# pkorus/neural-imaging

Hardware: AMD Instinct MI355X
Metric: patches/s (fwd+bwd) ISP->JPEG->FAN @256^2 (higher is better)
Workload: dtype bf16; 1 GPU; c4 = train_manipulation UNet->[native,sharpen:1,resample:50,gaussian:0.83,jpeg:80]->dJPEG(QF80,soft)->FAN, ds none, trainable nip+fan, lambda_nip 0.1; raw_patch=128, batch_per_gpu=64, global_batch=64, parallelism=dp1, world_size=1, hip_graph=False

## Files before the change

### include/nimg.h

```cpp
#ifndef NIMG_H
#define NIMG_H

#include <stddef.h>
#include <stdint.h>

#ifdef __cplusplus
extern "C" {
#endif

#define NIMG_OK 0
#define NIMG_ERR_ARG (-1)
#define NIMG_ERR_LAUNCH (-2)
#define NIMG_ERR_WORKSPACE (-3)

#define NIMG_BF16_IN 1
#define NIMG_BF16_OUT 2
#define NIMG_BF16_MASK 4
#define NIMG_BF16_DZ 8
#define NIMG_D2S_OUT 16
#define NIMG_MASK_CONV 128
#define NIMG_COPY_LRELU 64
#define NIMG_S2D_OUT 32
#define NIMG_UNPOOL_OUT 512
#define NIMG_D2S_CONVT 1024
#define NIMG_POOL_ALSO 256

#define NIMG_ABI_VERSION 8
int nimg_abi_version(void);

#define NIMG_ROUND_ROUND 0
#define NIMG_ROUND_SOFT 1
#define NIMG_ROUND_SIN 2
#define NIMG_ROUND_HARMONIC 3
#define NIMG_ROUND_IDENTITY 4

int nimg_djpeg_fwd(const float* x, float* y, const float* qtab, uint8_t* mask, int16_t* idx, float* xdq,
                   int n, int h, int w, int rounding, void* stream);
int nimg_djpeg_bwd(const float* x, const float* gy, const uint8_t* mask, const float* qtab, float* gx,
                   int n, int h, int w, int rounding, void* stream);
size_t nimg_djpeg_dq_workspace_bytes(int n, int h, int w);
int nimg_djpeg_bwd_dq(const float* x, const float* gy, const uint8_t* mask, const float* qtab, float* gx, float* dq,
                      int n, int h, int w, int rounding, int accumulate, void* workspace, size_t workspace_bytes,
                      void* stream);
size_t nimg_djpeg_sub_workspace_bytes(int n, int h, int w, int hs, int vs, int with_dq);
int nimg_djpeg_sub_fwd(const float* x, float* y, const float* qtab, uint8_t* mask, int16_t* idx, float* xdq,
                       int n, int h, int w, int hs, int vs, int rounding, void* workspace, size_t workspace_bytes,
                       void* stream);
int nimg_djpeg_sub_bwd(const float* x, const float* gy, const uint8_t* mask, const float* qtab, float* gx,
                       float* dq , int n, int h, int w, int hs, int vs, int rounding, int accumulate,
                       void* workspace, size_t workspace_bytes, void* stream);
int nimg_jpeg_qtable(int quality, int channel, float* out64);

int nimg_conv2d_fwd(const float* in1, int c1, const float* in2, int c2, const float* w, const float* bias,
                    float* out1, int o1, float* out2, int o2, const float* act_mask, int n, int h, int wd, int ks,
                    int stride, int pad_t, int pad_l, int pad_mode, int hout, int wout, int act, float alpha,
                    void* stream);
int nimg_conv_flip_weights(const float* w, float* wt, int ks_h, int ks_w, int cin, int cout, void* stream);
size_t nimg_conv2d_wgrad_workspace_bytes(int cin, int cout, int ks_h, int ks_w, int n, int hout, int wout);
int nimg_conv2d_wgrad(const float* in1, int c1, const float* in2, int c2, const float* dz, int cout, float* dw,
                      float* db, int n, int h, int wd, int ks, int stride, int pad_t, int pad_l, int pad_mode, int hout,
                      int wout, int accumulate, void* workspace, size_t workspace_bytes, void* stream);
size_t nimg_bias_grad_workspace_bytes(long npix, int cout);
int nimg_bias_grad(const float* dz, float* db, long npix, int cout, int accumulate, void* workspace,
                   size_t workspace_bytes, void* stream);
int nimg_bias_grad_ex(const float* dz, float* db, long npix, int cout, int accumulate, void* workspace,
                      size_t workspace_bytes, int flags, void* stream);
int nimg_convt2x2_fwd(const float* x, const float* w, const float* bias, float* y, int n, int h, int wd, int cin,
                      int cout, void* stream);

int nimg_maxpool2_fwd(const float* x, float* y, int n, int h, int w, int c, void* stream);
int nimg_maxpool2_bwd(const float* dp, const float* yact, const float* add, float* dz, int n, int h, int w, int c,
                      int apply_lrelu_mask, float alpha, void* stream);
int nimg_maxpool2_fwd_bf16(const void* x, void* y, int n, int h, int w, int c, void* stream);
int nimg_maxpool2_bwd_bf16(const void* dp, const void* yact, const void* add, void* dz, int n, int h, int w, int c,
                           int apply_lrelu_mask, float alpha, void* stream);
int nimg_conv2d_pool_fwd(const float* in, int cin, const float* w, const float* bias, float* pool_out,
                         unsigned char* pool_idx, int cout, int n, int h, int wd, int ks, int act, float alpha,
                         void* stream);
int nimg_conv2d_pool_fwd_bf16(const float* in, int cin, const float* w, const void* wb, const float* bias,
                              float* pool_out, unsigned char* pool_idx, int cout, int n, int h, int wd, int ks, int act,
                              float alpha, void* stream);
int nimg_maxpool2_unpool(const float* dp, const unsigned char* idx, const float* pooled, float* dz, int n, int ho, int wo,
                         int c, int apply_lrelu_mask, float alpha, void* stream);
int nimg_d2s_clip_fwd(const float* x, float* y, int n, int h, int w, int cout, float scale, float shift, int clip,
                      void* stream);
int nimg_d2s_clip_bwd(const float* dy, float* dx, int n, int h, int w, int cout, float scale, void* stream);
int nimg_lrelu_bwd(const float* dy, const float* yact, float* dz, long count, float alpha, void* stream);
int nimg_add(const float* a, const float* b, float* out, long count, void* stream);
int nimg_add_n(const float* const* inputs, int n_inputs, float* out, long count, void* stream);
int nimg_avgpool_fwd(const float* x, float* y, int n, int h, int w, int c, int factor, void* stream);
int nimg_avgpool_bwd(const float* dy, float* dx, int n, int h, int w, int c, int factor, void* stream);

size_t nimg_mse255_workspace_bytes(void);
int nimg_mse255(const float* a, const float* b, float* loss, float* grad_a, long count, float grad_scale,
                int accumulate, void* workspace, size_t workspace_bytes, void* stream);
size_t nimg_mae255_workspace_bytes(void);
int nimg_mae255(const float* a, const float* b, float* loss, float* grad_a, long count, float grad_scale,
                int accumulate, void* workspace, size_t workspace_bytes, void* stream);
size_t nimg_ssim_loss_workspace_bytes(int n, int h, int w, int c, int with_grad);
int nimg_ssim_loss(const float* y, const float* t, float* loss, float* grad_y, int n, int h, int w, int c,
                   float max_val, const float* gauss_win, float grad_scale, int accumulate, void* workspace,
                   size_t workspace_bytes, void* stream);
int nimg_mse255_sum_s2d3(const float* const* parts, int n_parts, const float* y, const float* target, float* loss, float* dz,
                         int n, int h, int w, float grad_scale, void* workspace, size_t workspace_bytes, void* stream);
size_t nimg_ssim_workspace_bytes(int n);
int nimg_ssim(const float* a, const float* b, float* out, int n, int h, int w, int c, int mode, float max_val,
              const float* gauss_win, void* workspace, size_t workspace_bytes, void* stream);
int nimg_fan_head_fwd(const float* act, const float* w, const float* b, const int* labels, float* gap, float* probs,
                      float* loss_per, float* dlogits, int n, int hw, int c, int k, float loss_scale, void* stream);
int nimg_fan_head_bwd(const float* act, const float* gap, const float* w, const float* dlogits,
                      const float* loss_per, float* dact, float* dw, float* db, float* loss, int n, int hw, int c,
                      int k, float loss_scale, float alpha, void* stream);
int nimg_adam_step(float* params, const float* grads, float* m, float* v, long count, float lr, float beta1,
                   float beta2, float eps, int step, float grad_scale, const int* skip_flag, void* stream);
int nimg_adam_step_dev(float* params, const float* grads, float* m, float* v, long count, const float* lr_t, float beta1,
                       float beta2, float eps, float grad_scale, const int* skip_flag, void* stream);
int nimg_nan_flag(const float* g, long count, int* flag, void* stream);
int nimg_int_words(int* dst, const int* src, long n, int value, int mode, void* stream);
int nimg_float_fill(float* dst, long n, float value, void* stream);

#define NIMG_TICKET_BYTES (64 * 1024)
#define NIMG_TICKET_STREAMS 16
int nimg_bind_tickets(void* stream, void* buf, size_t bytes);

int nimg_stream_create_cu_mask(int n_cus, void** stream);
int nimg_stream_destroy(void* stream);

int nimg_head_fused_ok(int hw, int c);
int nimg_head_fwd(const void* x, const void* wimg, const float* bias, unsigned* mask, unsigned* mask_p, float* gap, int n, int hw,
                  int c, float alpha, void* stream);
size_t nimg_head_wgrad_workspace_bytes(int n, int c);
int nimg_head_wgrad(const void* x, const unsigned* mask_p, const float* dlogits, const float* wdense, int k, float* dw, float* db,
                    int n, int hw, int c, float alpha, int accumulate, void* workspace, size_t workspace_bytes, void* stream);
int nimg_head_dgrad(const unsigned* mask, const float* dlogits, const float* wdense, int k, const void* wimg_t,
                    const void* in_mask, void* dx, int n, int hw, int c, float alpha, void* stream);
int nimg_head_dact(const unsigned* mask, const float* dlogits, const float* wdense, int k, void* dact, int n, int hw, int c,
                   float alpha, void* stream);
int nimg_fan_dense_fwd(const float* gap, const float* w, const float* b, const int* labels, float* probs, float* loss_per,
                       float* dlogits, int n, int c, int k, float loss_scale, void* stream);
int nimg_fan_dense_bwd(const float* gap, const float* dlogits, const float* loss_per, float* dw, float* db, float* loss, int n,
                       int c, int k, float loss_scale, void* stream);

int nimg_constrained_kernel_fwd(const float* kernel, float* nf, int ks, int channels, float strength, void* stream);
int nimg_constrained_kernel_bwd(const float* kernel, const float* dnf, float* dkernel, int ks, int channels,
                                float strength, void* stream);
int nimg_fold_pad(const float* dpad, float* dx, int n, int h, int w, int c, int pad, int pad_mode, void* stream);

int nimg_gaussian_fwd(const float* x, float* y, uint8_t* mask, const float* gk25, int n, int h, int w, int clip,
                      void* stream);
int nimg_gaussian_bwd(const float* dy, const uint8_t* mask, float* dx, const float* gk25, int n, int h, int w,
                      void* stream);
int nimg_dwfilter_fwd(const float* x, float* y, uint8_t* mask, const float* taps, int k, int pad_mode, int n, int h, int w,
                      int clip, void* stream);
int nimg_dwfilter_bwd(const float* dy, const uint8_t* mask, float* dx, const float* taps, int k, int pad_mode, int n, int h,
                      int w, void* stream);
int nimg_sharpen_fwd(const float* x, float* y, float* aux_hsv, uint8_t* mask, const float* gk9, int n, int h, int w,
                     void* stream);
int nimg_sharpen_bwd(const float* x, const float* dy, float* aux_hsv, const uint8_t* mask, float* dx,
                     const float* gk9, int n, int h, int w, void* stream);
int nimg_sparse_axis_apply(const float* in, float* out, const int* rowptr, const int* col, const float* val, int n,
                           int hin, int win, int c, int axis, int out_size, void* stream);

size_t nimg_ssim_planes_workspace_bytes(int n, int c);
int nimg_ssim_planes(const float* y, const float* t, int n, int h, int w, int c, float max_val, const float* gauss_win,
                     float* mean_ssim, float* mean_cs, float* maps, int which_maps, void* workspace,
                     size_t workspace_bytes, void* stream);
int nimg_msssim_combine(const float* values, const float* items, int scales, int planes, float* loss, float* coef,
                        void* stream);
int nimg_ssim_maps_grad(const float* y, const float* t, const float* maps, const float* coef, float* grad_y, int n,
                        int h, int w, int c, const float* gauss_win, float grad_scale, int accumulate, void* stream);
size_t nimg_msssim_workspace_bytes(int n, int h, int w, int c);
int nimg_msssim(const float* a, const float* b, int n, int h, int w, int c, float max_val, const float* gauss_win, double* out,
                void* workspace, size_t workspace_bytes, void* stream);

int nimg_patch_stats(const uint8_t* rgb, int n_images, int h, int w, const int* image_idx, const int* cand_xy, int b,
                     int attempts, int patch, double* var_out, double* mean_out, void* stream);
int nimg_patch_select(const int* cand_xy, const float* uniforms, const double* var, const double* mean, int b,
                      int attempts, int max_attempts, int mode, int* chosen_xy, int* attempts_used, void* stream);
int nimg_patch_gather(const uint16_t* raw, const uint8_t* rgb, int n_images, int h, int w, const int* image_idx,
                      const int* xy, int b, int patch, float* x_out, float* y_out, void* stream);

int nimg_affine(const float* x, float* y, long count, float a, float b, void* stream);
int nimg_lrelu_fwd(const float* x, float* y, long count, float alpha, void* stream);
int nimg_tanh_fwd(const float* x, float* y, long count, void* stream);
int nimg_tanh_bwd(const float* dy, const float* y, float* dx, long count, void* stream);
int nimg_clip01(const float* x, float* y, long count, void* stream);
int nimg_pad2d(const float* x, float* y, int n, int h, int w, int c, int pad, int pad_mode, void* stream);
int nimg_isp_residual_fwd(const float* x, const float* f, const float* alpha, float* y, long count, int clip,
                          void* stream);
long nimg_isp_residual_workspace_bytes(void);
int nimg_isp_residual_bwd(const float* dy, const float* f, const float* alpha, float* df, float* dalpha,
                          float* workspace, long count, int accumulate, void* stream);
int nimg_mask_scale(const float* x, const uint8_t* keep, float* y, long count, float scale, void* stream);
size_t nimg_conv5_dgrad_sparse_image_bytes(int cin, int cout);
int nimg_conv5_dgrad_sparse_weights(const float* w, void* image, int cin, int cout, void* stream);
int nimg_conv5_dgrad_sparse(const void* g, const unsigned char* idx, int cout, const void* image, void* out, int cin,
                            const void* act_mask, int n, int h, int wd, float alpha, int flags, void* stream);
int nimg_conv2d_fwd_bf16_res(const float* in1, int c1, const void* wb, const float* bias, float* out1, int o1,
                             const float* act_mask, const float* residual, void* out_bf16_copy, int n, int h, int wd, int ks,
                             int stride, int pad_t, int pad_l, int pad_mode, int hout, int wout, int act, float alpha, int flags,
                             void* stream);
int nimg_conv2d_fwd_bf16_unpool(const void* in_pooled, const unsigned char* in_idx, int c1, const void* wb, const float* bias,
                                float* out1, int o1, const float* act_mask, int n, int h, int w_, int ks, int pad_t, int pad_l,
                                int hout, int wout, int act, float alpha, int flags, void* stream);
int nimg_conv2d_wgrad_bf16_unpool(const void* in, int cin, const void* g, const unsigned char* idx, int cout, float* dw, float* db,
                                  int n, int h, int w_, int ks, int accumulate, void* workspace, size_t workspace_bytes,
                                  void* stream);
int nimg_conv2d_wgrad_bf16_deferred(const void* in1, int c1, const void* in2, int c2, const void* dz, const unsigned char* idx,
                                    int cout, float* dw, float* db, int n, int h, int wd, int ks, int stride, int pad_t, int pad_l,
                                    int pad_mode, int hout, int wout, void* workspace, size_t workspace_bytes, int flags,
                                    void* entry, void* stream);
int nimg_conv2d_wgrad_bf16_chained(const void* in1, int c1, const void* in2, int c2, const void* dz, const unsigned char* idx,
                                   int cout, float* dw, float* db, int n, int h, int wd, int ks, int stride, int pad_t, int pad_l,
                                   int pad_mode, int hout, int wout, void* workspace, size_t workspace_bytes, int flags,
                                   const void* pre_entry, void* entry, void* stream);
size_t nimg_reduce_entry_bytes(void);
int nimg_reduce_batch_max(void);
int nimg_reduce_slabs_batch(const void* entries, int n, void* stream);

int nimg_conv5c3_bf16(const float* in, const float* w, float* out, int n, int h, int wd, void* stream);
int nimg_cconv3(const float* in, const float* w, float* out_f32, void* out_c4, int n, int h, int w_, int pad_mode,
                void* stream);
int nimg_cconv3_dgrad_border(const float* dc, const float* nf, float* dx, int n, int h, int w_, void* stream);
int nimg_conv1_pool_fwd_c4(const void* c4, const float* w, const float* bias, void* pooled, unsigned char* pool_idx, int n,
                           int h, int w_, float alpha, int out_bf16, void* stream);
size_t nimg_conv1_wgrad_c4_workspace_bytes(void);
int nimg_conv1_wgrad_c4(const void* c4, const void* g, const unsigned char* pool_idx, float* dw, float* db, int n, int h, int w_,
                        int g_bf16, int accumulate, void* workspace, size_t workspace_bytes, void* stream);
int nimg_conv1_dgrad_pooled(const void* g, const unsigned char* pool_idx, const float* w, float* dc, int n, int h, int w_,
                            int g_bf16, void* stream);
int nimg_confusion_accumulate(const float* probs, const int* labels, int* pred, unsigned long long* conf, int n, int k,
                              void* stream);
int nimg_sigmoid_fwd(const float* x, float* y, long count, void* stream);
int nimg_sigmoid_bwd(const float* dy, const float* y, float* dx, long count, void* stream);
int nimg_activation_fwd(const float* x, float* y, long count, int kind, float alpha, void* stream);
int nimg_activation_bwd(const float* dy, const float* y, float* dx, long count, int kind, float alpha, void* stream);
int nimg_gamma_ste_fwd(const float* x, float* y, long count, float lo, float hi, float exponent, void* stream);
int nimg_gamma_ste_bwd(const float* x, const float* dy, float* dx, long count, float lo, float hi, float exponent,
                       void* stream);
int nimg_s2d2_affine_bf16(const float* x, void* y, int n, int h, int w, int c, int cp, float a, float b, void* stream);
int nimg_s2d_conv_weights(const float* w5, float* w3, int cin, int cp, int cout, void* stream);
int nimg_s2d_conv_weights_bwd(const float* dw3, float* dw5, int cin, int cp, int cout, int accumulate, void* stream);
int nimg_d2s2_scale(const float* xs, float* x, int n, int h, int w, int c, int cp, float scale, void* stream);
int nimg_zero_insert2(const float* in, float* out, int n, int h, int w, int c, void* stream);
size_t nimg_latent_workspace_bytes(int codebook_size);
int nimg_latent_fwd(const float* z, const float* scale, const float* codebook, int codebook_size, float v,
                    float gamma, int soft_codebook, float* latent, float* entropy, long count, long count_global,
                    void* workspace, size_t workspace_bytes, int finalize, void* stream);
int nimg_latent_entropy_finalize(int codebook_size, long count_global, float* entropy, void* workspace, void* stream);
int nimg_latent_bwd(const float* z, const float* scale, const float* latent, const float* dlatent,
                    float entropy_coef, const float* codebook, int codebook_size, float v, float gamma,
                    int soft_codebook, float* dz, float* dscale, int accumulate_dscale, long count, void* workspace,
                    size_t workspace_bytes, void* stream);
size_t nimg_l2_loss_workspace_bytes(void);
int nimg_l2_loss(const float* target, const float* y, float* loss, float* grad_y, long count, float grad_scale,
                 int accumulate, void* workspace, size_t workspace_bytes, void* stream);

size_t nimg_conv_weights_bf16_bytes(int ks_h, int ks_w, int cin, int cout, int mode);
int nimg_conv_weights_bf16(const float* w, void* wb, int ks_h, int ks_w, int cin, int cout, int mode, void* stream);
int nimg_conv2d_wgrad_pooled_bf16(const float* in, int cin, const float* g, const unsigned char* idx, int cout,
                                  float* dw, float* db, int n, int h, int wd, int ks, int accumulate, void* workspace,
                                  size_t workspace_bytes, void* stream);
int nimg_conv2d_dgrad_fewin_pooled_bf16(const float* g, const unsigned char* idx, const float* w, float* out, int ci,
                                        int cz, int n, int h, int wd, int ks, void* stream);
int nimg_conv2d_fwd_bf16_ex(const float* in1, int c1, const float* in2, int c2, const void* wb, const float* bias,
                            float* out1, int o1, float* out2, int o2, const float* act_mask, int n, int h, int wd,
                            int ks, int stride, int pad_t, int pad_l, int pad_mode, int hout, int wout, int act,
                            float alpha, int flags, void* stream);
int nimg_conv2d_wgrad_bf16_ex(const float* in1, int c1, const float* in2, int c2, const float* dz, int cout, float* dw,
                              float* db, int n, int h, int wd, int ks, int stride, int pad_t, int pad_l, int pad_mode,
                              int hout, int wout, int accumulate, void* workspace, size_t workspace_bytes, int flags,
                              void* stream);
int nimg_conv2d_pool_fwd_bf16_ex(const float* in, int cin, const float* w, const void* wb, const float* bias,
                                 float* pool_out, unsigned char* pool_idx, int cout, int n, int h, int wd, int ks,
                                 int act, float alpha, int flags, void* stream);
int nimg_conv2d_fwd_pool_also_bf16(const float* in, int cin, const void* wb, const float* bias, float* out, float* pool_out,
                                   unsigned char* pool_idx, int cout, int n, int h, int wd, int act, float alpha, void* stream);
#define NIMG_ROWS_F32_OUT 1
int nimg_conv3_rows_bf16(const void* in1, int c1, const void* in2, int c2, const void* wb, const float* bias, const void* mask,
                         void* out, void* out2, void* pool_out, int n, int h, int wd, int cout, int act, float alpha, int flags,
                         void* stream);
int nimg_conv3_rows_d2s_bf16(const void* in, int c1, const void* wb, const float* bias, float* y, int n, int h, int wd, void* stream);
int nimg_conv3_rows_c4_bf16(const float* in, const float* w, const float* bias, void* out, int n, int h, int wd, int act, float alpha,
                            void* stream);

int nimg_conv2d_dgrad_unpool_out_bf16(const float* dz, int c1, const void* wb, const float* act, const float* skip, float* out,
                                      int cout, int n, int h, int wd, int apply_mask, float alpha, void* stream);
int nimg_conv2d_wgrad_pooled_bf16_ex(const float* in, int cin, const float* g, const unsigned char* idx, int cout,
                                     float* dw, float* db, int n, int h, int wd, int ks, int accumulate, void* workspace,
                                     size_t workspace_bytes, int flags, void* stream);
int nimg_conv2d_dgrad_fewin_pooled_bf16_ex(const float* g, const unsigned char* idx, const float* w, float* out, int ci,
                                           int cz, int n, int h, int wd, int ks, int flags, void* stream);
int nimg_maxpool2_unpool_ex(const float* dp, const unsigned char* idx, const float* pooled, float* dz, int n, int ho,
                            int wo, int c, int apply_lrelu_mask, float alpha, int flags, void* stream);
int nimg_convt2x2_fwd_bf16(const float* x, const void* wb, const float* bias, float* y, int n, int h, int wd, int cin,
                           int cout, void* stream);
int nimg_convt2x2_fwd_bf16_ex(const float* x, const void* wb, const float* bias, float* y, int n, int h, int wd, int cin,
                              int cout, int flags, void* stream);
int nimg_conv_weights_bf16_batch(const void* table, int n_entries, void* stream);
int nimg_conv2d_fwd_bf16(const float* in1, int c1, const float* in2, int c2, const void* wb, const float* bias,
                         float* out1, int o1, float* out2, int o2, const float* act_mask, int n, int h, int wd,
                         int ks, int stride, int pad_t, int pad_l, int pad_mode, int hout, int wout, int act,
                         float alpha, void* stream);
size_t nimg_conv2d_wgrad_bf16_workspace_bytes(int cin, int cout, int ks_h, int ks_w, int n, int hout, int wout);
int nimg_conv2d_wgrad_bf16(const float* in1, int c1, const float* in2, int c2, const float* dz, int cout, float* dw,
                           float* db, int n, int h, int wd, int ks, int stride, int pad_t, int pad_l, int pad_mode,
                           int hout, int wout, int accumulate, void* workspace, size_t workspace_bytes, void* stream);

int nimg_conv2d_fwd_smallc_bf16(const float* in, int cin, const float* w, const float* bias, float* out, int cout,
                                int n, int h, int wd, int ks, int pad_mode, int act, float alpha, void* stream);
int nimg_conv2d_fwd_smallc_bf16_ex(const float* in, int cin, const float* w, const float* bias, float* out, int cout,
                                   int n, int h, int wd, int ks, int pad_mode, int act, float alpha, int flags, void* stream);
int nimg_conv2d_dgrad_fewin_bf16(const float* dz, const float* w, float* out, int ci, int cz, int n, int h, int wd,
                                 int ks, void* stream);

int nimg_awgn_fwd(const float* x, const float* noise, float* y, uint8_t* mask, long count, float strength,
                  void* stream);
int nimg_awgn_bwd(const float* x, const float* noise, const float* dy, const uint8_t* mask, float* dx, long count,
                  float strength, void* stream);
int nimg_gamma_fwd(const float* x, float* y, long count, float gamma, void* stream);
int nimg_gamma_bwd(const float* x, const float* dy, float* dx, long count, float gamma, void* stream);
int nimg_median_fwd(const float* x, float* y, uint8_t* sel, int n, int h, int w, int kernel, void* stream);
int nimg_median_bwd(const float* dy, const uint8_t* sel, float* dx, int n, int h, int w, int kernel, void* stream);

#define NIMG_L3IC_E_READ 1
#define NIMG_L3IC_E_LANES 2
#define NIMG_L3IC_E_RANGE 4
#define NIMG_L3IC_E_SYMBOL 8
#define NIMG_L3IC_E_FREQ 16
#define NIMG_L3IC_E_VARINT 32
#define NIMG_L3IC_E_ODD 64
#define NIMG_L3IC_E_UNUSED 128
#define NIMG_L3IC_E_STATE 256
#define NIMG_L3IC_E_RLE 512
size_t nimg_l3ic_workspace_bytes(int n_streams, int n_sym);
int nimg_l3ic_quantise(const float* z, const float* codebook, int codebook_size, uint8_t* idx, int* err, int n, int h,
                       int w, int c, void* stream);
int nimg_l3ic_encode(const uint8_t* idx, int n_streams, int n_sym, uint8_t* out, uint32_t* lengths, uint32_t* hist,
                     uint32_t* freq, void* workspace, size_t workspace_bytes, void* stream);
int nimg_l3ic_decode(const uint8_t* data, const uint32_t* offsets, const uint32_t* lengths, const float* codebook,
                     int codebook_size, float* z, uint32_t* err, int n, int h, int w, int c, void* stream);

size_t nimg_jpeg_workspace_bytes(int n, int h, int w, int hs, int vs);
int nimg_jpeg_transform(const void* x, int is_u8, int n, int h, int w, int hs, int vs, int quality, int16_t* coef, void* workspace,
                        size_t workspace_bytes, void* stream);
int nimg_jpeg_encode(const int16_t* coef, int n, int h, int w, int hs, int vs, uint8_t* out, size_t out_capacity, uint32_t* lengths,
// ... 57 lines not shown
```

### neural-imaging_amd/_lib.py

```python
import ctypes
import os
from ctypes import c_float, c_int, c_long, c_size_t, c_void_p

_HERE = os.path.dirname(os.path.abspath(__file__))
LIB_PATH = os.environ.get('NIMG_LIBPATH') or os.path.join(_HERE, 'libnimg.so')

P = c_void_p

PROTOTYPES = {
    'nimg_abi_version': (c_int, []),
    'nimg_djpeg_fwd': (c_int, [P, P, P, P, P, P, c_int, c_int, c_int, c_int, P]),
    'nimg_djpeg_bwd': (c_int, [P, P, P, P, P, c_int, c_int, c_int, c_int, P]),
    'nimg_djpeg_dq_workspace_bytes': (c_size_t, [c_int, c_int, c_int]),
    'nimg_djpeg_bwd_dq': (c_int, [P, P, P, P, P, P, c_int, c_int, c_int, c_int, c_int, P, c_size_t, P]),
    'nimg_djpeg_sub_workspace_bytes': (c_size_t, [c_int, c_int, c_int, c_int, c_int, c_int]),
    'nimg_djpeg_sub_fwd': (c_int, [P, P, P, P, P, P, c_int, c_int, c_int, c_int, c_int, c_int, P, c_size_t, P]),
    'nimg_djpeg_sub_bwd': (c_int, [P, P, P, P, P, P, c_int, c_int, c_int, c_int, c_int, c_int, c_int, P, c_size_t, P]),
    'nimg_jpeg_qtable': (c_int, [c_int, c_int, P]),
    'nimg_conv2d_fwd': (c_int, [P, c_int, P, c_int, P, P, P, c_int, P, c_int, P, c_int, c_int, c_int, c_int, c_int,
                                c_int, c_int, c_int, c_int, c_int, c_int, c_float, P]),
    'nimg_conv_flip_weights': (c_int, [P, P, c_int, c_int, c_int, c_int, P]),
    'nimg_conv2d_wgrad_workspace_bytes': (c_size_t, [c_int, c_int, c_int, c_int, c_int, c_int, c_int]),
    'nimg_conv2d_wgrad': (c_int, [P, c_int, P, c_int, P, c_int, P, P, c_int, c_int, c_int, c_int, c_int, c_int, c_int,
                                  c_int, c_int, c_int, c_int, P, c_size_t, P]),
    'nimg_bias_grad_workspace_bytes': (c_size_t, [c_long, c_int]),
    'nimg_bias_grad': (c_int, [P, P, c_long, c_int, c_int, P, c_size_t, P]),
    'nimg_bias_grad_ex': (c_int, [P, P, c_long, c_int, c_int, P, c_size_t, c_int, P]),
    'nimg_convt2x2_fwd': (c_int, [P, P, P, P, c_int, c_int, c_int, c_int, c_int, P]),
    'nimg_maxpool2_fwd': (c_int, [P, P, c_int, c_int, c_int, c_int, P]),
    'nimg_maxpool2_bwd': (c_int, [P, P, P, P, c_int, c_int, c_int, c_int, c_int, c_float, P]),
    'nimg_maxpool2_fwd_bf16': (c_int, [P, P, c_int, c_int, c_int, c_int, P]),
    'nimg_maxpool2_bwd_bf16': (c_int, [P, P, P, P, c_int, c_int, c_int, c_int, c_int, c_float, P]),
    'nimg_conv2d_pool_fwd': (c_int, [P, c_int, P, P, P, P, c_int, c_int, c_int, c_int, c_int, c_int, c_float, P]),
    'nimg_conv2d_pool_fwd_bf16': (c_int, [P, c_int, P, P, P, P, P, c_int, c_int, c_int, c_int, c_int, c_int, c_float,
                                          P]),
    'nimg_maxpool2_unpool': (c_int, [P, P, P, P, c_int, c_int, c_int, c_int, c_int, c_float, P]),
    'nimg_d2s_clip_fwd': (c_int, [P, P, c_int, c_int, c_int, c_int, c_float, c_float, c_int, P]),
    'nimg_d2s_clip_bwd': (c_int, [P, P, c_int, c_int, c_int, c_int, c_float, P]),
    'nimg_lrelu_bwd': (c_int, [P, P, P, c_long, c_float, P]),
    'nimg_add': (c_int, [P, P, P, c_long, P]),
    'nimg_add_n': (c_int, [P, c_int, P, c_long, P]),
    'nimg_avgpool_fwd': (c_int, [P, P, c_int, c_int, c_int, c_int, c_int, P]),
    'nimg_avgpool_bwd': (c_int, [P, P, c_int, c_int, c_int, c_int, c_int, P]),
    'nimg_mse255_workspace_bytes': (c_size_t, []),
    'nimg_mse255': (c_int, [P, P, P, P, c_long, c_float, c_int, P, c_size_t, P]),
    'nimg_mse255_sum_s2d3': (c_int, [P, c_int, P, P, P, P, c_int, c_int, c_int, c_float, P, c_size_t, P]),
    'nimg_fan_head_fwd': (c_int, [P, P, P, P, P, P, P, P, c_int, c_int, c_int, c_int, c_float, P]),
    'nimg_fan_head_bwd': (c_int, [P, P, P, P, P, P, P, P, P, c_int, c_int, c_int, c_int, c_float, c_float, P]),
    'nimg_adam_step': (c_int, [P, P, P, P, c_long, c_float, c_float, c_float, c_float, c_int, c_float, P, P]),
    'nimg_adam_step_dev': (c_int, [P, P, P, P, c_long, P, c_float, c_float, c_float, c_float, P, P]),
    'nimg_conv3_rows_bf16': (c_int, [P, c_int, P, c_int, P, P, P, P, P, P, c_int, c_int, c_int, c_int, c_int, c_float, c_int, P]),
    'nimg_conv3_rows_d2s_bf16': (c_int, [P, c_int, P, P, P, c_int, c_int, c_int, P]),
    'nimg_conv2d_wgrad_bf16_deferred': (c_int, [P, c_int, P, c_int, P, P, c_int, P, P, c_int, c_int, c_int, c_int, c_int, c_int, c_int,
                                                c_int, c_int, c_int, P, c_size_t, c_int, P, P]),
    'nimg_conv2d_wgrad_bf16_chained': (c_int, [P, c_int, P, c_int, P, P, c_int, P, P, c_int, c_int, c_int, c_int, c_int, c_int, c_int,
                                               c_int, c_int, c_int, P, c_size_t, c_int, P, P, P]),
    'nimg_reduce_entry_bytes': (c_size_t, []),
    'nimg_reduce_batch_max': (c_int, []),
    'nimg_reduce_slabs_batch': (c_int, [P, c_int, P]),
    'nimg_conv3_rows_c4_bf16': (c_int, [P, P, P, P, c_int, c_int, c_int, c_int, c_float, P]),
    'nimg_nan_flag': (c_int, [P, c_long, P, P]),
    'nimg_int_words': (c_int, [P, P, c_long, c_int, c_int, P]),
    'nimg_float_fill': (c_int, [P, c_long, c_float, P]),
    'nimg_bind_tickets': (c_int, [P, P, c_size_t]),
    'nimg_stream_create_cu_mask': (c_int, [c_int, P]),
    'nimg_stream_destroy': (c_int, [P]),
    'nimg_head_fused_ok': (c_int, [c_int, c_int]),
    'nimg_head_fwd': (c_int, [P, P, P, P, P, P, c_int, c_int, c_int, c_float, P]),
    'nimg_head_wgrad_workspace_bytes': (c_size_t, [c_int, c_int]),
    'nimg_head_wgrad': (c_int, [P, P, P, P, c_int, P, P, c_int, c_int, c_int, c_float, c_int, P, c_size_t, P]),
    'nimg_head_dgrad': (c_int, [P, P, P, c_int, P, P, P, c_int, c_int, c_int, c_float, P]),
    'nimg_head_dact': (c_int, [P, P, P, c_int, P, c_int, c_int, c_int, c_float, P]),
    'nimg_fan_dense_fwd': (c_int, [P, P, P, P, P, P, P, c_int, c_int, c_int, c_float, P]),
    'nimg_fan_dense_bwd': (c_int, [P, P, P, P, P, P, c_int, c_int, c_int, c_float, P]),
    'nimg_constrained_kernel_fwd': (c_int, [P, P, c_int, c_int, c_float, P]),
    'nimg_constrained_kernel_bwd': (c_int, [P, P, P, c_int, c_int, c_float, P]),
    'nimg_fold_pad': (c_int, [P, P, c_int, c_int, c_int, c_int, c_int, c_int, P]),
    'nimg_gaussian_fwd': (c_int, [P, P, P, P, c_int, c_int, c_int, c_int, P]),
    'nimg_gaussian_bwd': (c_int, [P, P, P, P, c_int, c_int, c_int, P]),
    'nimg_dwfilter_fwd': (c_int, [P, P, P, P, c_int, c_int, c_int, c_int, c_int, c_int, P]),
    'nimg_dwfilter_bwd': (c_int, [P, P, P, P, c_int, c_int, c_int, c_int, c_int, P]),
    'nimg_sharpen_fwd': (c_int, [P, P, P, P, P, c_int, c_int, c_int, P]),
    'nimg_sharpen_bwd': (c_int, [P, P, P, P, P, P, c_int, c_int, c_int, P]),
    'nimg_affine': (c_int, [P, P, c_long, c_float, c_float, P]),
    'nimg_lrelu_fwd': (c_int, [P, P, c_long, c_float, P]),
    'nimg_zero_insert2': (c_int, [P, P, c_int, c_int, c_int, c_int, P]),
    'nimg_s2d2_affine_bf16': (c_int, [P, P, c_int, c_int, c_int, c_int, c_int, c_float, c_float, P]),
    'nimg_s2d_conv_weights': (c_int, [P, P, c_int, c_int, c_int, P]),
    'nimg_s2d_conv_weights_bwd': (c_int, [P, P, c_int, c_int, c_int, c_int, P]),
    'nimg_d2s2_scale': (c_int, [P, P, c_int, c_int, c_int, c_int, c_int, c_float, P]),
    'nimg_latent_workspace_bytes': (c_size_t, [c_int]),
    'nimg_latent_fwd': (c_int, [P, P, P, c_int, c_float, c_float, c_int, P, P, c_long, c_long, P, c_size_t, c_int, P]),
    'nimg_latent_entropy_finalize': (c_int, [c_int, c_long, P, P, P]),
    'nimg_latent_bwd': (c_int, [P, P, P, P, c_float, P, c_int, c_float, c_float, c_int, P, P, c_int, c_long, P,
                                c_size_t, P]),
    'nimg_l2_loss_workspace_bytes': (c_size_t, []),
    'nimg_l2_loss': (c_int, [P, P, P, P, c_long, c_float, c_int, P, c_size_t, P]),
    'nimg_conv_weights_bf16_bytes': (c_size_t, [c_int, c_int, c_int, c_int, c_int]),
    'nimg_conv_weights_bf16': (c_int, [P, P, c_int, c_int, c_int, c_int, c_int, P]),
    'nimg_conv2d_fwd_bf16': (c_int, [P, c_int, P, c_int, P, P, P, c_int, P, c_int, P, c_int, c_int, c_int, c_int,
                                     c_int, c_int, c_int, c_int, c_int, c_int, c_int, c_float, P]),
    'nimg_conv2d_wgrad_bf16_workspace_bytes': (c_size_t, [c_int, c_int, c_int, c_int, c_int, c_int, c_int]),
    'nimg_conv2d_wgrad_bf16': (c_int, [P, c_int, P, c_int, P, c_int, P, P, c_int, c_int, c_int, c_int, c_int, c_int,
                                       c_int, c_int, c_int, c_int, c_int, P, c_size_t, P]),
    'nimg_conv2d_wgrad_pooled_bf16': (c_int, [P, c_int, P, P, c_int, P, P, c_int, c_int, c_int, c_int, c_int, P, c_size_t,
                                              P]),
    'nimg_conv2d_dgrad_fewin_pooled_bf16': (c_int, [P, P, P, P, c_int, c_int, c_int, c_int, c_int, c_int, P]),
    'nimg_ssim_workspace_bytes': (c_size_t, [c_int]),
    'nimg_ssim': (c_int, [P, P, P, c_int, c_int, c_int, c_int, c_int, c_float, P, P, c_size_t, P]),
    'nimg_tanh_fwd': (c_int, [P, P, c_long, P]),
    'nimg_tanh_bwd': (c_int, [P, P, P, c_long, P]),
    'nimg_clip01': (c_int, [P, P, c_long, P]),
    'nimg_isp_residual_fwd': (c_int, [P, P, P, P, c_long, c_int, P]),
    'nimg_isp_residual_workspace_bytes': (c_long, []),
    'nimg_isp_residual_bwd': (c_int, [P, P, P, P, P, P, c_long, c_int, P]),
    'nimg_activation_fwd': (c_int, [P, P, c_long, c_int, c_float, P]),
    'nimg_activation_bwd': (c_int, [P, P, P, c_long, c_int, c_float, P]),
    'nimg_sigmoid_fwd': (c_int, [P, P, c_long, P]),
    'nimg_sigmoid_bwd': (c_int, [P, P, P, c_long, P]),
    'nimg_gamma_ste_fwd': (c_int, [P, P, c_long, c_float, c_float, c_float, P]),
    'nimg_gamma_ste_bwd': (c_int, [P, P, P, c_long, c_float, c_float, c_float, P]),
    'nimg_mae255_workspace_bytes': (c_size_t, []),
    'nimg_mae255': (c_int, [P, P, P, P, c_long, c_float, c_int, P, c_size_t, P]),
    'nimg_ssim_loss_workspace_bytes': (c_size_t, [c_int, c_int, c_int, c_int, c_int]),
    'nimg_ssim_loss': (c_int, [P, P, P, P, c_int, c_int, c_int, c_int, c_float, P, c_float, c_int, P, c_size_t, P]),
    'nimg_patch_stats': (c_int, [P, c_int, c_int, c_int, P, P, c_int, c_int, c_int, P, P, P]),
    'nimg_patch_select': (c_int, [P, P, P, P, c_int, c_int, c_int, c_int, P, P, P]),
    'nimg_patch_gather': (c_int, [P, P, c_int, c_int, c_int, P, P, c_int, c_int, P, P, P]),
    'nimg_mask_scale': (c_int, [P, P, P, c_long, c_float, P]),
    'nimg_conv5_dgrad_sparse_image_bytes': (c_size_t, [c_int, c_int]),
    'nimg_conv5_dgrad_sparse_weights': (c_int, [P, P, c_int, c_int, P]),
    'nimg_conv5_dgrad_sparse': (c_int, [P, P, c_int, P, P, c_int, P, c_int, c_int, c_int, c_float, c_int, P]),
    'nimg_conv2d_fwd_bf16_res': (c_int, [P, c_int, P, P, P, c_int, P, P, P, c_int, c_int, c_int, c_int, c_int, c_int, c_int, c_int, c_int,
                                 c_int, c_int, c_float, c_int, P]),
    'nimg_conv2d_fwd_bf16_unpool': (c_int, [P, P, c_int, P, P, P, c_int, P, c_int, c_int, c_int, c_int, c_int, c_int, c_int,
                                            c_int, c_int, c_float, c_int, P]),
    'nimg_conv2d_wgrad_bf16_unpool': (c_int, [P, c_int, P, P, c_int, P, P, c_int, c_int, c_int, c_int, c_int, P, c_size_t, P]),
    'nimg_cconv3': (c_int, [P, P, P, P, c_int, c_int, c_int, c_int, P]),
    'nimg_conv5c3_bf16': (c_int, [P, P, P, c_int, c_int, c_int, P]),
    'nimg_cconv3_dgrad_border': (c_int, [P, P, P, c_int, c_int, c_int, P]),
    'nimg_conv1_pool_fwd_c4': (c_int, [P, P, P, P, P, c_int, c_int, c_int, c_float, c_int, P]),
    'nimg_conv1_wgrad_c4_workspace_bytes': (c_size_t, []),
    'nimg_conv1_wgrad_c4': (c_int, [P, P, P, P, P, c_int, c_int, c_int, c_int, c_int, P, c_size_t, P]),
    'nimg_conv1_dgrad_pooled': (c_int, [P, P, P, P, c_int, c_int, c_int, c_int, P]),
    'nimg_confusion_accumulate': (c_int, [P, P, P, P, c_int, c_int, P]),
    'nimg_ssim_planes_workspace_bytes': (c_size_t, [c_int, c_int]),
    'nimg_ssim_planes': (c_int, [P, P, c_int, c_int, c_int, c_int, c_float, P, P, P, P, c_int, P, c_size_t, P]),
    'nimg_msssim_combine': (c_int, [P, P, c_int, c_int, P, P, P]),
    'nimg_ssim_maps_grad': (c_int, [P, P, P, P, P, c_int, c_int, c_int, c_int, P, c_float, c_int, P]),
    'nimg_pad2d': (c_int, [P, P, c_int, c_int, c_int, c_int, c_int, c_int, P]),
    'nimg_conv2d_fwd_bf16_ex': (c_int, [P, c_int, P, c_int, P, P, P, c_int, P, c_int, P, c_int, c_int, c_int, c_int, c_int,
                                        c_int, c_int, c_int, c_int, c_int, c_int, c_float, c_int, P]),
    'nimg_conv2d_wgrad_bf16_ex': (c_int, [P, c_int, P, c_int, P, c_int, P, P, c_int, c_int, c_int, c_int, c_int, c_int,
                                          c_int, c_int, c_int, c_int, c_int, P, c_size_t, c_int, P]),
    'nimg_conv2d_pool_fwd_bf16_ex': (c_int, [P, c_int, P, P, P, P, P, c_int, c_int, c_int, c_int, c_int, c_int, c_float,
                                             c_int, P]),
    'nimg_conv2d_dgrad_unpool_out_bf16': (c_int, [P, c_int, P, P, P, P, c_int, c_int, c_int, c_int, c_int, c_float, P]),
    'nimg_conv2d_fwd_pool_also_bf16': (c_int, [P, c_int, P, P, P, P, P, c_int, c_int, c_int, c_int, c_int, c_float, P]),
    'nimg_conv2d_wgrad_pooled_bf16_ex': (c_int, [P, c_int, P, P, c_int, P, P, c_int, c_int, c_int, c_int, c_int, P,
                                                 c_size_t, c_int, P]),
    'nimg_conv2d_dgrad_fewin_pooled_bf16_ex': (c_int, [P, P, P, P, c_int, c_int, c_int, c_int, c_int, c_int, c_int, P]),
    'nimg_maxpool2_unpool_ex': (c_int, [P, P, P, P, c_int, c_int, c_int, c_int, c_int, c_float, c_int, P]),
    'nimg_conv_weights_bf16_batch': (c_int, [P, c_int, P]),
    'nimg_convt2x2_fwd_bf16': (c_int, [P, P, P, P, c_int, c_int, c_int, c_int, c_int, P]),
    'nimg_convt2x2_fwd_bf16_ex': (c_int, [P, P, P, P, c_int, c_int, c_int, c_int, c_int, c_int, P]),
    'nimg_conv2d_fwd_smallc_bf16': (c_int, [P, c_int, P, P, P, c_int, c_int, c_int, c_int, c_int, c_int, c_int,
                                            c_float, P]),
    'nimg_conv2d_fwd_smallc_bf16_ex': (c_int, [P, c_int, P, P, P, c_int, c_int, c_int, c_int, c_int, c_int, c_int,
                                               c_float, c_int, P]),
    'nimg_conv2d_dgrad_fewin_bf16': (c_int, [P, P, P, c_int, c_int, c_int, c_int, c_int, c_int, P]),
    'nimg_awgn_fwd': (c_int, [P, P, P, P, c_long, c_float, P]),
    'nimg_awgn_bwd': (c_int, [P, P, P, P, P, c_long, c_float, P]),
    'nimg_gamma_fwd': (c_int, [P, P, c_long, c_float, P]),
    'nimg_gamma_bwd': (c_int, [P, P, P, c_long, c_float, P]),
    'nimg_median_fwd': (c_int, [P, P, P, c_int, c_int, c_int, c_int, P]),
    'nimg_median_bwd': (c_int, [P, P, P, c_int, c_int, c_int, c_int, P]),
    'nimg_sparse_axis_apply': (c_int, [P, P, P, P, P, c_int, c_int, c_int, c_int, c_int, c_int, P]),
    'nimg_l3ic_workspace_bytes': (c_size_t, [c_int, c_int]),
    'nimg_l3ic_quantise': (c_int, [P, P, c_int, P, P, c_int, c_int, c_int, c_int, P]),
    'nimg_l3ic_encode': (c_int, [P, c_int, c_int, P, P, P, P, P, c_size_t, P]),
    'nimg_l3ic_decode': (c_int, [P, P, P, P, c_int, P, P, c_int, c_int, c_int, c_int, P]),
    'nimg_jpeg_workspace_bytes': (c_size_t, [c_int, c_int, c_int, c_int, c_int]),
    'nimg_jpeg_transform': (c_int, [P, c_int, c_int, c_int, c_int, c_int, c_int, c_int, P, P, c_size_t, P]),
    'nimg_jpeg_encode': (c_int, [P, c_int, c_int, c_int, c_int, c_int, P, c_size_t, P, P, c_size_t, P]),
    'nimg_jpeg_reconstruct': (c_int, [P, c_int, c_int, c_int, c_int, c_int, c_int, P, P, c_size_t, P]),
    'nimg_jpeg_transform_items': (c_int, [P, c_int, c_int, c_int, c_int, c_int, c_int, P, c_int, P, P, P, c_size_t, P]),
    'nimg_jpeg_reconstruct_items': (c_int, [P, c_int, c_int, c_int, c_int, c_int, P, P, P, P, c_size_t, P]),
    'nimg_jpeg_decode_workspace_bytes': (c_size_t, [c_int, c_int, c_int, c_int, c_int, c_size_t, c_int]),
    'nimg_jpeg_decode': (c_int, [P, P, P, c_int, c_int, c_int, c_int, c_int, c_int, P, P, P, P, c_size_t, P]),
    'nimg_jpeg_reconstruct_tables': (c_int, [P, c_int, c_int, c_int, c_int, c_int, P, P, c_int, P, c_size_t, P]),
    'nimg_jpeg_histogram': (c_int, [P, c_int, c_int, c_int, c_int, c_int, P, P]),
    'nimg_jpeg_optimal_tables': (c_int, [P, c_int, P, P, P]),
    'nimg_jpeg_encode_tables_workspace_bytes': (c_size_t, [c_int, c_int, c_int, c_int, c_int]),
    'nimg_jpeg_encode_tables': (c_int, [P, c_int, c_int, c_int, c_int, c_int, P, P, c_size_t, P, P, P, c_size_t, P]),
    'nimg_jpeg_transform_tables': (c_int, [P, c_int, c_int, c_int, c_int, c_int, c_int, P, c_int, P, P, P, c_size_t, P]),
    'nimg_jpeg_tables_from_float': (c_int, [P, c_int, c_int, P, P, P]),
    'nimg_jpeg_encode_restart_workspace_bytes': (c_size_t, [c_int, c_int, c_int, c_int, c_int, c_int]),
    'nimg_jpeg_encode_restart': (c_int, [P, c_int, c_int, c_int, c_int, c_int, c_int, P, c_size_t, P, P, c_size_t, P]),
    'nimg_jpeg_histogram_restart': (c_int, [P, c_int, c_int, c_int, c_int, c_int, c_int, P, P]),
    'nimg_jpeg_encode_tables_restart_workspace_bytes': (c_size_t, [c_int, c_int, c_int, c_int, c_int, c_int]),
    'nimg_jpeg_encode_tables_restart': (c_int, [P, c_int, c_int, c_int, c_int, c_int, c_int, P, P, c_size_t, P, P, P, c_size_t, P]),
    'nimg_jpeg_decode_restart_workspace_bytes': (c_size_t, [c_int, c_int, c_int, c_int, c_int, c_int, c_size_t, c_int]),
    'nimg_jpeg_decode_restart': (c_int, [P, P, P, c_int, c_int, c_int, c_int, c_int, c_int, c_int, P, P, P, P, c_size_t, P]),
    'nimg_msssim_workspace_bytes': (c_size_t, [c_int, c_int, c_int, c_int]),
    'nimg_msssim': (c_int, [P, P, c_int, c_int, c_int, c_int, c_float, P, P, P, c_size_t, P]),
    'nimg_conv1_pool_fwd_c4_sign': (c_int, [P, P, P, P, P, P, c_int, c_int, c_int, c_float, c_int, P]),
    'nimg_conv2d_pool_sign_ok': (c_int, [c_int, c_int, c_int, c_int, c_int, c_int, c_int]),
    'nimg_conv2d_pool_fwd_bf16_sign': (c_int, [P, c_int, P, P, P, P, P, P, c_int, c_int, c_int, c_int, c_int, c_int, c_float,
                                               c_int, P]),
    'nimg_conv2d_fwd_bf16_unpool_sign': (c_int, [P, P, c_int, P, P, P, c_int, P, P, c_int, c_int, c_int, c_int, c_int, c_int, c_int,
                                                 c_int, c_int, c_float, c_int, P]),
}

ERRORS = {-1: 'NIMG_ERR_ARG (invalid argument / unsupported configuration)',
          -2: 'NIMG_ERR_LAUNCH (HIP kernel launch failed)',
          -3: 'NIMG_ERR_WORKSPACE (workspace too small)'}

_lib = None


ABI_VERSION = 8
TICKET_BYTES = 64 * 1024


def load():
    global _lib
    if _lib is not None:
        return _lib
    if not os.path.isfile(LIB_PATH):
        raise RuntimeError('libnimg.so not found at {} - build it with neural-imaging_amd/csrc/build.sh '
                           '(or __graft_entry__.build()); there is no CPU fallback'.format(LIB_PATH))
    import torch
    lib = ctypes.CDLL(LIB_PATH)
    for name, (res, args) in PROTOTYPES.items():
        fn = getattr(lib, name)
        fn.restype = res
        fn.argtypes = args
    if lib.nimg_abi_version() != ABI_VERSION:
        raise RuntimeError('libnimg.so at {} has ABI version {}, this binding was written against {} - rebuild it '
                           '(neural-imaging_amd/csrc/build.sh)'.format(LIB_PATH, lib.nimg_abi_version(), ABI_VERSION))
    _lib = lib
    return lib


def call(name, *args):
    rc = getattr(load(), name)(*args)
    if rc != 0:
        raise RuntimeError('{} failed: {}'.format(name, ERRORS.get(rc, rc)))
    return rc
```

### neural-imaging_amd/csrc/djpeg.h

```cpp
#pragma once
#include <type_traits>
#include "common.h"

namespace nimg {
namespace dj {

constexpr int STRIP_PX = 64;
constexpr int ROW_STRIDE = 196;
constexpr int STAGE_F = 8 * ROW_STRIDE;

__device__ __forceinline__ void wave_sync() { __builtin_amdgcn_wave_barrier(); }

__device__ constexpr float kF[8][8] = {
    {0.3536f, 0.3536f, 0.3536f, 0.3536f, 0.3536f, 0.3536f, 0.3536f, 0.3536f},
    {0.4904f, 0.4157f, 0.2778f, 0.0975f, -0.0975f, -0.2778f, -0.4157f, -0.4904f},
    {0.4619f, 0.1913f, -0.1913f, -0.4619f, -0.4619f, -0.1913f, 0.1913f, 0.4619f},
    {0.4157f, -0.0975f, -0.4904f, -0.2778f, 0.2778f, 0.4904f, 0.0975f, -0.4157f},
    {0.3536f, -0.3536f, -0.3536f, 0.3536f, 0.3536f, -0.3536f, -0.3536f, 0.3536f},
    {0.2778f, -0.4904f, 0.0975f, 0.4157f, -0.4157f, -0.0975f, 0.4904f, -0.2778f},
    {0.1913f, -0.4619f, 0.4619f, -0.1913f, -0.1913f, 0.4619f, -0.4619f, 0.1913f},
    {0.0975f, -0.2778f, 0.4157f, -0.4904f, 0.4904f, -0.4157f, 0.2778f, -0.0975f}};

__device__ constexpr float kCF[3][4] = {{0.0f, 0.299f, 0.587f, 0.114f},
                                        {128.0f, -0.168736f, -0.331264f, 0.5f},
                                        {128.0f, 0.5f, -0.418688f, -0.081312f}};
__device__ constexpr float kCI[3][4] = {{(float)(-1.402 * 128), 1.0f, 0.0f, 1.402f},
                                        {(float)(1.058272 * 128), 1.0f, -0.344136f, -0.714136f},
                                        {(float)(-1.772 * 128), 1.0f, 1.772f, 0.0f}};

__device__ __forceinline__ void dct_fwd8(const float (&in)[8], float (&out)[8]) {
#pragma unroll
    for (int k = 0; k < 8; ++k) {
        float acc = in[0] * kF[k][0];
#pragma unroll
        for (int m = 1; m < 8; ++m) acc = __builtin_fmaf(in[m], kF[k][m], acc);
        out[k] = acc;
    }
}
__device__ __forceinline__ void dct_inv8(const float (&in)[8], float (&out)[8]) {
#pragma unroll
    for (int m = 0; m < 8; ++m) {
        float acc = in[0] * kF[0][m];
#pragma unroll
        for (int k = 1; k < 8; ++k) acc = __builtin_fmaf(in[k], kF[k][m], acc);
        out[m] = acc;
    }
}

struct Task {
    int n, by, x0;
    bool valid;
};

__device__ __forceinline__ Task decode_task(long task, long n_tasks, int hb, int strips) {
    Task t;
    t.valid = task < n_tasks;
    const long tt = t.valid ? task : 0;
    t.x0 = (int)(tt % strips) * STRIP_PX;
    t.by = (int)((tt / strips) % hb);
    t.n = (int)(tt / ((long)strips * hb));
    return t;
}

typedef float f32x4 __attribute__((ext_vector_type(4)));
__device__ __forceinline__ void fetch_strip(const float* __restrict__ src, f32x4 (&pre)[6], const Task& t, int h, int w,
                                            int lane) {
    const int strip_f = min(STRIP_PX, w - t.x0) * 3;
#pragma unroll
    for (int it = 0; it < 6; ++it) {
        const int idx = it * 64 + lane;
        const int row = idx / 48, c4 = idx % 48;
        if (t.valid && c4 * 4 < strip_f)
            pre[it] = *reinterpret_cast<const f32x4*>(src + (((long)t.n * h + t.by * 8 + row) * w + t.x0) * 3 + c4 * 4);
    }
}
__device__ __forceinline__ void commit_strip(float* lds, const f32x4 (&pre)[6], int lane) {
#pragma unroll
    for (int it = 0; it < 6; ++it) {
        const int idx = it * 64 + lane;
        *reinterpret_cast<f32x4*>(lds + (idx / 48) * ROW_STRIDE + (idx % 48) * 4) = pre[it];
    }
}

__device__ __forceinline__ void store_strip(float* __restrict__ dst, const float* lds, const Task& t, int h, int w,
                                            int lane) {
    const int strip_f = min(STRIP_PX, w - t.x0) * 3;
#pragma unroll
    for (int it = 0; it < 6; ++it) {
        const int idx = it * 64 + lane;
        const int row = idx / 48, c4 = idx % 48;
        if (t.valid && c4 * 4 < strip_f) {
            const float4 v = *reinterpret_cast<const float4*>(lds + row * ROW_STRIDE + c4 * 4);
            *reinterpret_cast<float4*>(dst + (((long)t.n * h + t.by * 8 + row) * w + t.x0) * 3 + c4 * 4) = v;
        }
    }
}

__device__ __forceinline__ void read_row24(const float* lds, int b, int r, float (&px)[24]) {
    const float4* p = reinterpret_cast<const float4*>(lds + r * ROW_STRIDE + b * 24);
#pragma unroll
    for (int k = 0; k < 6; ++k) {
        const float4 v = p[k];
        px[4 * k + 0] = v.x; px[4 * k + 1] = v.y; px[4 * k + 2] = v.z; px[4 * k + 3] = v.w;
    }
}
__device__ __forceinline__ void write_row24(float* lds, int b, int r, const float (&px)[24]) {
    float4* p = reinterpret_cast<float4*>(lds + r * ROW_STRIDE + b * 24);
#pragma unroll
    for (int k = 0; k < 6; ++k) p[k] = make_float4(px[4 * k], px[4 * k + 1], px[4 * k + 2], px[4 * k + 3]);
}

template <int NC>
__device__ __forceinline__ void transpose_tiles(float* tile, int b, int r, float (&v)[NC][8]) {
#pragma unroll
    for (int c = 0; c < NC; ++c)
#pragma unroll
        for (int k = 0; k < 8; ++k) tile[((c * 8 + b) * 8 + r) * 9 + k] = v[c][k];
    wave_sync();
#pragma unroll
    for (int c = 0; c < NC; ++c)
#pragma unroll
        for (int k = 0; k < 8; ++k) v[c][k] = tile[((c * 8 + b) * 8 + k) * 9 + r];
    wave_sync();
}

enum { Q_RINT = 0, Q_SIN = 1, Q_HARMONIC = 2, Q_IDENTITY = 3 };
__host__ __device__ constexpr int fwd_mode(int rounding) {
    return rounding == NIMG_ROUND_SIN ? Q_SIN : rounding == NIMG_ROUND_HARMONIC ? Q_HARMONIC
         : rounding == NIMG_ROUND_IDENTITY ? Q_IDENTITY : Q_RINT;
}
template <int QMODE>
__device__ __forceinline__ float quantise(float u) {
    if constexpr (QMODE == Q_RINT) return rintf(u);
    else if constexpr (QMODE == Q_SIN) return u - sinpif(2.0f * (u - rintf(u))) * 0.15915494309189535f;
    else if constexpr (QMODE == Q_HARMONIC) return u - sinpif(2.0f * (u - rintf(u))) * 0.3183098861837907f;
    else return u;
}
enum { G_ZERO = 0, G_SOFT = 1, G_HARMONIC = 2, G_ONE = 3 };
__host__ __device__ constexpr int bwd_mode(int rounding) {
    return rounding == NIMG_ROUND_ROUND ? G_ZERO : rounding == NIMG_ROUND_HARMONIC ? G_HARMONIC
         : rounding == NIMG_ROUND_IDENTITY ? G_ONE : G_SOFT;
}
template <int GMODE>
__device__ __forceinline__ float quantise_grad(float u) {
    if constexpr (GMODE == G_ZERO) return 0.0f;
    else if constexpr (GMODE == G_ONE) return 1.0f;
    else {
        const float c = __builtin_amdgcn_cosf(__builtin_amdgcn_fractf(u));
        return GMODE == G_SOFT ? 1.0f - c : 1.0f - 2.0f * c;
    }
}

template <bool EXACT>
__device__ __forceinline__ float div_q(float x, float q, float rc) {
    if constexpr (EXACT) return x / q;
    const float y0 = x * rc;
    const float r = __builtin_fmaf(-y0, q, x);
    return __builtin_fmaf(r, rc, y0);
}

__device__ __forceinline__ void colour_fwd(const float (&px)[24], float (&ycc)[3][8]) {
#pragma unroll
    for (int j = 0; j < 8; ++j) {
        const float r = 255.0f * px[3 * j], g = 255.0f * px[3 * j + 1], bb = 255.0f * px[3 * j + 2];
#pragma unroll
        for (int c = 0; c < 3; ++c) {
            float acc = kCF[c][0];
            acc = __builtin_fmaf(r, kCF[c][1], acc);
            acc = __builtin_fmaf(g, kCF[c][2], acc);
            acc = __builtin_fmaf(bb, kCF[c][3], acc);
            ycc[c][j] = acc - 127.0f;
        }
    }
}

__device__ __forceinline__ bool stage_tables(const float* __restrict__ qtab, float* qT, int* flag) {
    const int tid = threadIdx.x;
    if (tid == 0) *flag = 1;
    __syncthreads();
    if (tid < 192) {
        const float q = qtab[tid];
        const int c = tid >> 6, u = (tid >> 3) & 7, r = tid & 7;
        qT[(c * 8 + r) * 8 + u] = q;
        qT[192 + (c * 8 + r) * 8 + u] = 1.0f / q;
        if (!(q >= 1.0f && q <= 255.0f && q == rintf(q))) *flag = 0;
    }
    __syncthreads();
    return __builtin_amdgcn_readfirstlane(*flag) != 0;
}
__device__ __forceinline__ void read_tables(const float* qT, int c, int r, float (&q)[8], float (&rc)[8]) {
#pragma unroll
    for (int k = 0; k < 2; ++k) {
        const float4 a = *reinterpret_cast<const float4*>(qT + (c * 8 + r) * 8 + 4 * k);
        const float4 b = *reinterpret_cast<const float4*>(qT + 192 + (c * 8 + r) * 8 + 4 * k);
        q[4 * k] = a.x; q[4 * k + 1] = a.y; q[4 * k + 2] = a.z; q[4 * k + 3] = a.w;
        rc[4 * k] = b.x; rc[4 * k + 1] = b.y; rc[4 * k + 2] = b.z; rc[4 * k + 3] = b.w;
    }
}

}
}
```

### neural-imaging_amd/csrc/djpeg.hip

```cpp
#include "djpeg.h"

namespace {

using namespace nimg;
using namespace nimg::dj;

constexpr int TILE_F = 3 * 8 * 72;
constexpr int WAVE_LDS_F = (STAGE_F > TILE_F ? STAGE_F : TILE_F);
constexpr int WAVES_PER_BLOCK = 4;
#ifndef DJ_FWD_WGS
#define DJ_FWD_WGS 4
#endif
#ifndef DJ_BWD_WGS
#define DJ_BWD_WGS 3
#endif

__device__ __forceinline__ void transpose24(float* tile, int b, int r, float (&v)[3][8]) { transpose_tiles<3>(tile, b, r, v); }

template <int QMODE, bool EXACT>
__device__ __forceinline__ void quantise_columns(float (&v)[3][8], const float* qT, const Task& t, int b, int r, int hb, int wb,
                                                 int16_t* __restrict__ idx, float* __restrict__ xdq) {
#pragma unroll
    for (int c = 0; c < 3; ++c) {
        float X[8], q[8], rc[8];
        dct_fwd8(v[c], X);
        read_tables(qT, c, r, q, rc);
#pragma unroll
        for (int u = 0; u < 8; ++u) {
            const float qi = quantise<QMODE>(div_q<EXACT>(X[u], q[u], rc[u]));
            X[u] = qi * q[u];
            if (idx || xdq) {
                const long o = ((((long)t.n * 3 + c) * hb + t.by) * wb + (t.x0 / 8 + b)) * 64 + u * 8 + r;
                if (idx) idx[o] = (int16_t)qi;
                if (xdq) xdq[o] = X[u];
            }
        }
        dct_inv8(X, v[c]);
    }
}

template <int QMODE>
__global__ __launch_bounds__(256, DJ_FWD_WGS) void djpeg_fwd_kernel(const float* __restrict__ x, float* __restrict__ y,
                                                        const float* __restrict__ qtab, uint8_t* __restrict__ mask,
                                                        int16_t* __restrict__ idx, float* __restrict__ xdq, int n,
                                                        int h, int w) {
    extern __shared__ __attribute__((aligned(16))) float smem[];
    const int wave = threadIdx.x >> 6, lane = threadIdx.x & 63;
    const int b = lane >> 3, r = lane & 7;
    float* lds = smem + wave * WAVE_LDS_F;
    float* qT = smem + WAVES_PER_BLOCK * WAVE_LDS_F;
    const int hb = h / 8, wb = w / 8, strips = (w + STRIP_PX - 1) / STRIP_PX;
    const long n_tasks = (long)n * hb * strips;
    const Task t = decode_task((long)blockIdx.x * WAVES_PER_BLOCK + wave, n_tasks, hb, strips);
    const bool active = t.valid && (t.x0 + b * 8 < w);
    constexpr float kRc255 = 1.0f / 255.0f;

    f32x4 pre[6] = {};
    fetch_strip(x, pre, t, h, w, lane);
    const bool fast = stage_tables(qtab, qT, reinterpret_cast<int*>(qT + 384));
    commit_strip(lds, pre, lane);
    wave_sync();
    float px[24];
    float v[3][8];
    read_row24(lds, b, r, px);
    wave_sync();
    {
        float ycc[3][8];
        colour_fwd(px, ycc);
#pragma unroll
        for (int c = 0; c < 3; ++c) dct_fwd8(ycc[c], v[c]);
    }
    transpose24(lds, b, r, v);
    if (active) {
        if (fast) quantise_columns<QMODE, false>(v, qT, t, b, r, hb, wb, idx, xdq);
        else quantise_columns<QMODE, true>(v, qT, t, b, r, hb, wb, idx, xdq);
    }
    transpose24(lds, b, r, v);
    {
        float q3[3][8];
#pragma unroll
        for (int c = 0; c < 3; ++c) {
            dct_inv8(v[c], q3[c]);
#pragma unroll
            for (int j = 0; j < 8; ++j) q3[c][j] += 127.0f;
        }
        uint32_t mlo = 0, mhi = 0;
#pragma unroll
        for (int j = 0; j < 8; ++j) {
            uint32_t m = 0;
#pragma unroll
            for (int c = 0; c < 3; ++c) {
                float acc = kCI[c][0];
                acc = __builtin_fmaf(q3[0][j], kCI[c][1], acc);
                acc = __builtin_fmaf(q3[1][j], kCI[c][2], acc);
                acc = __builtin_fmaf(q3[2][j], kCI[c][3], acc);
                acc = div_q<false>(acc, 255.0f, kRc255);
                const float cl = __builtin_amdgcn_fmed3f(acc, 0.0f, 1.0f);
                m |= cl == acc ? (1u << c) : 0u;
                px[3 * j + c] = cl;
            }
            if (j < 4) mlo |= m << (8 * j); else mhi |= m << (8 * (j - 4));
        }
        write_row24(lds, b, r, px);
        if (mask && active)
            *reinterpret_cast<uint2*>(mask + ((long)t.n * h + t.by * 8 + r) * w + t.x0 + b * 8) = make_uint2(mlo, mhi);
    }
    wave_sync();
    store_strip(y, lds, t, h, w, lane);
}

template <int RND, bool DQ>
__global__ __launch_bounds__(256, DQ ? 3 : DJ_BWD_WGS) void djpeg_bwd_kernel(const float* __restrict__ x, const float* __restrict__ gy,
                                                        const uint8_t* __restrict__ mask,
                                                        const float* __restrict__ qtab, float* __restrict__ gx,
                                                        float* __restrict__ dq_partial, int n, int h, int w) {
    constexpr int GMODE = bwd_mode(RND), QMODE = fwd_mode(RND);
    extern __shared__ __attribute__((aligned(16))) float smem[];
    const int wave = threadIdx.x >> 6, lane = threadIdx.x & 63;
    const int b = lane >> 3, r = lane & 7;
    float* lds = smem + wave * WAVE_LDS_F;
    float* qT = smem + WAVES_PER_BLOCK * WAVE_LDS_F;
    const int hb = h / 8, strips = (w + STRIP_PX - 1) / STRIP_PX;
    const long n_tasks = (long)n * hb * strips;
    const Task t = decode_task((long)blockIdx.x * WAVES_PER_BLOCK + wave, n_tasks, hb, strips);
    const bool active = t.valid && (t.x0 + b * 8 < w);
    f32x4 pre[6] = {};
    fetch_strip(x, pre, t, h, w, lane);
    const bool fast = stage_tables(qtab, qT, reinterpret_cast<int*>(qT + 384)) && !DQ;

    float px[24];
    float tx[3][8];
    float tg[3][8];
    commit_strip(lds, pre, lane);
    fetch_strip(gy, pre, t, h, w, lane);
    uint2 mm = make_uint2(0u, 0u);
    if (active) mm = *reinterpret_cast<const uint2*>(mask + ((long)t.n * h + t.by * 8 + r) * w + t.x0 + b * 8);
    wave_sync();
    read_row24(lds, b, r, px);
    wave_sync();
    {
        float ycc[3][8];
        colour_fwd(px, ycc);
#pragma unroll
        for (int c = 0; c < 3; ++c) dct_fwd8(ycc[c], tx[c]);
    }
    commit_strip(lds, pre, lane);
    wave_sync();
    read_row24(lds, b, r, px);
    wave_sync();
    {
#pragma clang fp contract(fast)
        float gq[3][8];
#pragma unroll
        for (int j = 0; j < 8; ++j) {
            const uint32_t m = ((j < 4 ? mm.x >> (8 * j) : mm.y >> (8 * (j - 4)))) & 0xffu;
            float g[3];
#pragma unroll
            for (int c = 0; c < 3; ++c) g[c] = (m >> c) & 1u ? px[3 * j + c] * (1.0f / 255.0f) : 0.0f;
#pragma unroll
            for (int c = 0; c < 3; ++c)
                gq[c][j] = g[0] * kCI[0][1 + c] + g[1] * kCI[1][1 + c] + g[2] * kCI[2][1 + c];
        }
#pragma unroll
        for (int c = 0; c < 3; ++c) dct_fwd8(gq[c], tg[c]);
    }
    transpose24(lds, b, r, tx);
    transpose24(lds, b, r, tg);
    float dqa[DQ ? 2 : 1][8];
    if constexpr (DQ) {
#pragma unroll
        for (int k = 0; k < 2; ++k)
#pragma unroll
            for (int u = 0; u < 8; ++u) dqa[k][u] = 0.0f;
    }
    if (active) {
        auto columns = [&](auto exact) {
#pragma unroll
            for (int c = 0; c < 3; ++c) {
                float X[8], G[8], q[8], rc[8];
                dct_fwd8(tx[c], X);
                dct_fwd8(tg[c], G);
                read_tables(qT, c, r, q, rc);
#pragma unroll
                for (int u = 0; u < 8; ++u) {
                    const float z = div_q<decltype(exact)::value>(X[u], q[u], rc[u]);
                    const float qg = quantise_grad<GMODE>(z);
                    if constexpr (DQ) dqa[c == 0 ? 0 : 1][u] += G[u] * (quantise<QMODE>(z) - z * qg);
                    G[u] *= qg;
                }
                dct_inv8(G, tg[c]);
            }
        };
        if (fast) columns(std::false_type{});
        else columns(std::true_type{});
    }
    if constexpr (DQ) {
        const long task = (long)blockIdx.x * WAVES_PER_BLOCK + wave;
#pragma unroll
        for (int k = 0; k < 2; ++k)
#pragma unroll
            for (int u = 0; u < 8; ++u) {
                float v = dqa[k][u];
                v += __shfl_xor(v, 8, 64);
                v += __shfl_xor(v, 16, 64);
                v += __shfl_xor(v, 32, 64);
                if (lane < 8) dq_partial[task * 128 + (k * 8 + u) * 8 + r] = v;
            }
    }
    transpose24(lds, b, r, tg);
    {
#pragma clang fp contract(fast)
        float gb[3][8];
#pragma unroll
        for (int c = 0; c < 3; ++c) dct_inv8(tg[c], gb[c]);
#pragma unroll
        for (int j = 0; j < 8; ++j)
#pragma unroll
            for (int c = 0; c < 3; ++c)
                px[3 * j + c] =
                    255.0f * (gb[0][j] * kCF[0][1 + c] + gb[1][j] * kCF[1][1 + c] + gb[2][j] * kCF[2][1 + c]);
        write_row24(lds, b, r, px);
    }
    wave_sync();
    store_strip(gx, lds, t, h, w, lane);
}

inline int persistent_grid(long tasks) { return (int)((tasks + WAVES_PER_BLOCK - 1) / WAVES_PER_BLOCK); }
constexpr size_t kLds = ((size_t)WAVES_PER_BLOCK * WAVE_LDS_F + 384 + 4) * sizeof(float);

template <bool DQ, typename... A>
void launch_bwd(int rounding, int grid, hipStream_t s, A... a) {
    const dim3 g(grid), b(256);
    switch (rounding) {
        case NIMG_ROUND_ROUND: hipLaunchKernelGGL((djpeg_bwd_kernel<NIMG_ROUND_ROUND, DQ>), g, b, kLds, s, a...); break;
        case NIMG_ROUND_SIN:
            if constexpr (DQ) { hipLaunchKernelGGL((djpeg_bwd_kernel<NIMG_ROUND_SIN, DQ>), g, b, kLds, s, a...); break; }
            [[fallthrough]];
        case NIMG_ROUND_SOFT: hipLaunchKernelGGL((djpeg_bwd_kernel<NIMG_ROUND_SOFT, DQ>), g, b, kLds, s, a...); break;
        case NIMG_ROUND_HARMONIC: hipLaunchKernelGGL((djpeg_bwd_kernel<NIMG_ROUND_HARMONIC, DQ>), g, b, kLds, s, a...); break;
        default: hipLaunchKernelGGL((djpeg_bwd_kernel<NIMG_ROUND_IDENTITY, DQ>), g, b, kLds, s, a...); break;
    }
}

}

extern "C" {

int nimg_abi_version(void) { return NIMG_ABI_VERSION; }

int nimg_djpeg_fwd(const float* x, float* y, const float* qtab, uint8_t* mask, int16_t* idx, float* xdq, int n,
                   int h, int w, int rounding, void* stream) {
    if (n == 0) return NIMG_OK;
    if (!x || !y || !qtab || n < 0 || h <= 0 || w <= 0 || (h % 8) || (w % 8)) return NIMG_ERR_ARG;
    if (rounding < NIMG_ROUND_ROUND || rounding > NIMG_ROUND_IDENTITY) return NIMG_ERR_ARG;
    if (n == 0) return NIMG_OK;
    const long tasks = (long)n * (h / 8) * ((w + STRIP_PX - 1) / STRIP_PX);
    const dim3 grid(persistent_grid(tasks)), block(256);
    hipStream_t s = (hipStream_t)stream;
    switch (fwd_mode(rounding)) {
        case Q_RINT: hipLaunchKernelGGL(djpeg_fwd_kernel<Q_RINT>, grid, block, kLds, s, x, y, qtab, mask, idx, xdq, n, h, w); break;
        case Q_SIN: hipLaunchKernelGGL(djpeg_fwd_kernel<Q_SIN>, grid, block, kLds, s, x, y, qtab, mask, idx, xdq, n, h, w); break;
        case Q_HARMONIC:
            hipLaunchKernelGGL(djpeg_fwd_kernel<Q_HARMONIC>, grid, block, kLds, s, x, y, qtab, mask, idx, xdq, n, h, w);
            break;
        default: hipLaunchKernelGGL(djpeg_fwd_kernel<Q_IDENTITY>, grid, block, kLds, s, x, y, qtab, mask, idx, xdq, n, h, w); break;
    }
    NIMG_CHECK_LAUNCH();
    return NIMG_OK;
}

int nimg_djpeg_bwd(const float* x, const float* gy, const uint8_t* mask, const float* qtab, float* gx, int n, int h,
                   int w, int rounding, void* stream) {
    if (n == 0) return NIMG_OK;
    if (!x || !gy || !mask || !qtab || !gx || n < 0 || h <= 0 || w <= 0 || (h % 8) || (w % 8)) return NIMG_ERR_ARG;
    if (rounding < NIMG_ROUND_ROUND || rounding > NIMG_ROUND_IDENTITY) return NIMG_ERR_ARG;
    if (n == 0) return NIMG_OK;
    const long tasks = (long)n * (h / 8) * ((w + STRIP_PX - 1) / STRIP_PX);
    launch_bwd<false>(rounding, persistent_grid(tasks), (hipStream_t)stream, x, gy, mask, qtab, gx, (float*)nullptr, n, h, w);
    NIMG_CHECK_LAUNCH();
    return NIMG_OK;
}

size_t nimg_djpeg_dq_workspace_bytes(int n, int h, int w) {
    if (n <= 0 || h <= 0 || w <= 0) return 0;
    const long tasks = (long)n * (h / 8) * ((w + STRIP_PX - 1) / STRIP_PX);
    return (size_t)nimg::cdiv(tasks, WAVES_PER_BLOCK) * WAVES_PER_BLOCK * 128 * sizeof(float);
}

int nimg_djpeg_bwd_dq(const float* x, const float* gy, const uint8_t* mask, const float* qtab, float* gx, float* dq,
                      int n, int h, int w, int rounding, int accumulate, void* workspace, size_t workspace_bytes,
                      void* stream) {
    if (n == 0) return NIMG_OK;
    if (!x || !gy || !mask || !qtab || !gx || !dq || !workspace || n < 0 || h <= 0 || w <= 0 || (h % 8) || (w % 8))
        return NIMG_ERR_ARG;
    if (rounding < NIMG_ROUND_ROUND || rounding > NIMG_ROUND_IDENTITY) return NIMG_ERR_ARG;
    if (workspace_bytes < nimg_djpeg_dq_workspace_bytes(n, h, w)) return NIMG_ERR_WORKSPACE;
    const long tasks = (long)n * (h / 8) * ((w + STRIP_PX - 1) / STRIP_PX);
    const int grid = persistent_grid(tasks);
    launch_bwd<true>(rounding, grid, (hipStream_t)stream, x, gy, mask, qtab, gx, (float*)workspace, n, h, w);
    NIMG_CHECK_LAUNCH();
    nimg::launch_reduce2((const float*)workspace, dq, 128, grid * WAVES_PER_BLOCK, nullptr, nullptr, 0, 0, accumulate,
                         (hipStream_t)stream);
    NIMG_CHECK_LAUNCH();
    return NIMG_OK;
}

int nimg_jpeg_qtable(int quality, int channel, float* out64) {
    static const float luma[64] = {16, 11, 10, 16, 24, 40, 51, 61, 12, 12, 14, 19, 26, 58, 60, 55,
                                   14, 13, 16, 24, 40, 57, 69, 56, 14, 17, 22, 29, 51, 87, 80, 62,
                                   18, 22, 37, 56, 68, 109, 103, 77, 24, 35, 55, 64, 81, 104, 113, 92,
                                   49, 64, 78, 87, 103, 121, 120, 101, 72, 92, 95, 98, 112, 100, 103, 99};
    static const float chroma[64] = {17, 18, 24, 47, 99, 99, 99, 99, 18, 21, 26, 66, 99, 99, 99, 99,
                                     24, 26, 56, 99, 99, 99, 99, 99, 47, 66, 99, 99, 99, 99, 99, 99,
                                     99, 99, 99, 99, 99, 99, 99, 99, 99, 99, 99, 99, 99, 99, 99, 99,
                                     99, 99, 99, 99, 99, 99, 99, 99, 99, 99, 99, 99, 99, 99, 99, 99};
    if (!out64) return NIMG_ERR_ARG;
    quality = quality > 100 ? 100 : (quality < 1 ? 1 : quality);
    const float s = quality < 50 ? (float)(5000.0 / quality) : (float)(200 - 2 * quality);
    const float* t = channel == 0 ? luma : chroma;
    for (int k = 0; k < 64; ++k) {
        float v = __builtin_floorf((t[k] * s + 50.0f) / 100.0f);
        out64[k] = v < 1.0f ? 1.0f : (v > 255.0f ? 255.0f : v);
    }
    return NIMG_OK;
}

}
```

### neural-imaging_amd/models/jpeg.py

```python
import numpy as np
import torch

from .. import ops
from ..device import DeviceArray, default_device, to_device
from ..helpers.utils import is_number
from ..compression.jpeg_helpers import compress_batch, device_codec, encode_batch, jpeg_qf_estimation, libjpeg_qtable
from .tfmodel import ParamStore, TFModel

_common_codec = None


def is_valid_quality(quality):
    if is_number(quality) and 1 <= quality <= 100:
        return True
    elif hasattr(quality, '__getitem__') and len(quality) > 1 and all((1 <= x <= 100) for x in quality):
        return True
    return False


def differentiable_jpeg(x, quality):
    global _common_codec
    if _common_codec is None:
        _common_codec = JPEG(None, 'soft')
    return _common_codec.process(x, quality)


class DifferentiableJPEG(object):

    def __init__(self, quality=None, rounding_approximation='sin', rounding_approximation_steps=5, trainable=False,
                 device=None, subsampling='4:4:4'):
        self.subsampling = subsampling
        self.factors = ops.jpeg_subsampling(subsampling)
        if quality is not None and not is_valid_quality(quality):
            raise ValueError('Invalid JPEG quality: requires int in [1,100] or an iterable with least 2 such numbers')
        if rounding_approximation is not None and rounding_approximation not in ['sin', 'harmonic', 'soft']:
            raise ValueError('Unsupported rounding approximation: {}'.format(rounding_approximation))
        self.quality = quality
        self.trainable = trainable
        self.rounding_approximation = rounding_approximation
        self.rounding_approximation_steps = rounding_approximation_steps
        self.device = device
        self._q_cache = {}
        self.params = None
        if trainable:
            self.params = ParamStore([('Q_mtx_luma', (8, 8)), ('Q_mtx_chroma', (8, 8))],
                                     device if device is not None else default_device())
            init = ops.qtables_device(quality if is_number(quality) else None, 'cpu')
            self.params.p['Q_mtx_luma'].copy_(init[0])
            self.params.p['Q_mtx_chroma'].copy_(init[1])

    def qtables(self, quality, device):
        key = (quality if is_number(quality) else None, str(device))
        if key not in self._q_cache:
            self._q_cache[key] = ops.qtables_device(key[0], device)
        return self._q_cache[key]

    def trainable_tables(self):
        return self.params.flat.view(2, 8, 8)[[0, 1, 1]].contiguous()

    def __call__(self, x, quality=None):
        q = self.trainable_tables() if (self.trainable and (quality is None or quality == self.quality)) else \
            self.qtables(self.quality if quality is None else quality, x.device)
        if self.factors != (1, 1):
            y, _, _, xdq = ops.djpeg_sub_fwd(x, q, self.rounding_approximation, *self.factors, want_mask=False, want_xdq=True)
            return y, xdq
        y, _, _, xdq = ops.djpeg_fwd(x, q, self.rounding_approximation, want_mask=False, want_xdq=True)
        return y, xdq


class JPEG(TFModel):

    def __init__(self, quality=None, codec='soft', trainable=False, device=None, subsampling='4:4:4'):
        super().__init__(device=device)
        if codec is not None and codec not in ['libjpeg', 'soft', 'sin', 'harmonic']:
            raise ValueError('Unsupported codec version: {}'.format(codec))
        self.subsampling = subsampling
        self._factors = ops.jpeg_subsampling(subsampling)
        self._codec_model = None if codec == 'libjpeg' else DifferentiableJPEG(quality, codec, trainable=trainable,
                                                                               device=self.device, subsampling=subsampling)
        self._model = self._codec_model.params if (trainable and self._codec_model is not None) else ParamStore([], self.device)
        self.trainable = bool(trainable)
        self.codec = codec
        self.quality = quality
        self.loss = self._mse

    def _mse(self, y_true, y_pred, sample_weight=None):
        a, b = to_device(y_true, self.device), to_device(y_pred, self.device)
        return float(DeviceArray(ops.mse255(a, b)[0])) / (255.0 * 255.0)

    def reset_performance_stats(self):
        self.performance = self._reset_performance(['entropy', 'ssim', 'psnr'])

    @staticmethod
    def resolve_quality(quality):
        if not is_valid_quality(quality):
            raise ValueError('Invalid or unspecified JPEG quality!')
        if hasattr(quality, '__getitem__') and len(quality) > 2:
            return int(np.random.choice(quality))
        elif hasattr(quality, '__getitem__') and len(quality) == 2:
            return int(np.random.randint(quality[0], quality[1]))
        elif is_number(quality) and 1 <= quality <= 100:
            return int(quality)
        raise ValueError('Invalid quality! {}'.format(quality))

    def forward(self, x, quality=None, training=False, out=None):
        if self._codec_model is None:
            if training:
                raise NotImplementedError('the libjpeg codec has no gradient (the reference has none either): train on a '
                                          'differentiable codec, validate on this one')
            y, _ = device_codec(x, self.resolve_quality(self.quality if quality is None else quality), self.subsampling,
                                want_bytes=False)
            if out is not None:
                out.copy_(y)
                y = out
            return y, None
        resolved = self.resolve_quality(self.quality if quality is None else quality)
        learned = bool(self.trainable) and is_number(self.quality) and resolved == self.quality
        if learned:
            q = self._codec_model.trainable_tables()
        else:
            q = self._codec_model.qtables(resolved, x.device)
        if self._factors != (1, 1):
            y, mask, _, _ = ops.djpeg_sub_fwd(x, q, self.codec, *self._factors, want_mask=training, out=out)
        else:
            y, mask, _, _ = ops.djpeg_fwd(x, q, self.codec, want_mask=training, out=out)
        return y, ({'x': x, 'mask': mask, 'q': q, 'learned': learned} if training else None)

    def backward(self, ctx, dy, accumulate=False):
        if self._codec_model is None:
            raise NotImplementedError('the libjpeg codec has no gradient')
        if self._factors != (1, 1):
            if ctx.get('learned'):
                return ops.djpeg_sub_bwd(ctx['x'], dy, ctx['mask'], ctx['q'], self.codec, *self._factors,
                                         dq=self._model.flat_grad, accumulate=accumulate)
            return ops.djpeg_sub_bwd(ctx['x'], dy, ctx['mask'], ctx['q'], self.codec, *self._factors)
        if ctx.get('learned'):
            return ops.djpeg_bwd(ctx['x'], dy, ctx['mask'], ctx['q'], self.codec, dq=self._model.flat_grad, accumulate=accumulate)
        return ops.djpeg_bwd(ctx['x'], dy, ctx['mask'], ctx['q'], self.codec)

    def process(self, batch_x, quality=None, return_entropy=False):
        y, _ = self.forward(to_device(batch_x, self.device), quality)
        y = DeviceArray(y)
        return (y, np.nan) if return_entropy else y

    def file_tables(self):
        if self._codec_model is None:
            if not is_number(self.quality):
                raise ValueError('file_tables needs a numeric quality with codec="libjpeg", got {}'.format(self.quality))
            q = self.resolve_quality(self.quality)
            return np.stack([libjpeg_qtable(q, c).ravel() for c in (0, 1)]).astype(np.uint16), np.zeros((2, 64), bool)
        if self.trainable:
            t = self._codec_model.params.flat.detach().view(1, 2, 64)
        else:
            t = self._codec_model.qtables(self.quality, self.device)[:2].reshape(1, 2, 64)
        t = t.contiguous()
        qtabs, _ = ops.jpeg_tables_from_float(t)
        both = torch.cat([qtabs[0, :2].reshape(-1).float(), t.reshape(-1)]).cpu().numpy()
        tables, t = both[:128].reshape(2, 64).astype(np.uint16), both[128:].reshape(2, 64)
        with np.errstate(invalid='ignore'):
            return tables, ~np.isfinite(t) | (np.rint(t) < 1) | (np.rint(t) > 255)

    def process_files(self, batch_x, subsampling=None, optimize=False, return_files=False):
        x = to_device(batch_x, self.device)
        if isinstance(x, torch.Tensor) and x.requires_grad:
            raise NotImplementedError('the real codec has no gradient (the reference has none either): train on a differentiable '
                                      'codec, measure on this one')
        tables, _ = self.file_tables()
        if subsampling is None:
            subsampling = self.subsampling
        y, sizes = compress_batch(x, None, subsampling=subsampling, optimize=optimize, qtables=tables)
        if y.ndim == 3:
            raise ValueError('process_files needs an (n,h,w,3) batch')
        if return_files:
            return y, sizes, encode_batch(x, None, subsampling, optimize=optimize, qtables=tables)
        return y, sizes

    def __repr__(self):
        sub = '' if self._factors == (1, 1) else ',subsampling="{}"'.format(self.subsampling)
        if self._codec_model is not None:
            return 'JPEG(quality={},codec="{}",trainable={}{})'.format(self.quality, self.codec, bool(self.trainable), sub)
        return 'JPEG(quality={},codec="{}"{})'.format(self.quality, self.codec, sub)

    def _sub_suffix(self):
        return '' if self._factors == (1, 1) else ' ' + self.subsampling

    def summary(self, quality=None):
        return 'JPEG ({}) {}{}'.format(self.codec, self._quality_mode(quality), self._sub_suffix())

    def summary_compact(self, quality=None):
        return 'JPEG ({}) {}{}'.format(self.codec, self._quality_mode(quality), self._sub_suffix())

    def _model_tables(self):
        if self.trainable:
            t = self._codec_model.params.flat.detach().cpu().view(2, 8, 8).numpy()
            return t[0], t[1]
        q = self._codec_model.qtables(self.quality, torch.device('cpu')).numpy()
        return q[0], q[1]

    def estimate_qf(self, channel=0):
        return jpeg_qf_estimation(self._model_tables()[0], channel)

    def _quality_mode(self, quality=None):
        quality = quality or self.quality
        if self.trainable and self._codec_model is not None:
            luma, chroma = self._model_tables()
            return 'trainable QF~{}/{}'.format(jpeg_qf_estimation(luma, 0), jpeg_qf_estimation(chroma, 1))
        elif is_number(quality):
            return 'QF={}'.format(quality)
        elif hasattr(quality, '__getitem__') and len(quality) == 2:
            return 'QF~[{},{}]'.format(*quality)
        elif hasattr(quality, '__getitem__') and len(quality) > 2:
            return 'QF~{{{}}}'.format(','.join(str(x) for x in quality))
        return 'QF=?'
```

### neural-imaging_amd/ops.py

```python
import math
import os

import numpy as np
import torch

from . import _lib

LRELU_ALPHA = 0.2

COMPUTE = 'f32'


STORE_BF16 = True


def set_compute(mode):
    global COMPUTE
    if mode not in ('f32', 'bf16'):
        raise ValueError('compute mode must be f32 or bf16')
    COMPUTE = mode


_WB_REGISTRY = {}

# ... 132 lines not shown
        nbytes = max(int(nbytes), 256)
        if self.buf is None or self.buf.numel() < nbytes or self.buf.device != device:
            self.buf = torch.empty(nbytes, dtype=torch.uint8, device=device)
        return pin(self.buf)

    arena, used, pending = None, 0, ()

    def claim(self, nbytes, device):
        nbytes = (max(int(nbytes), 256) + 255) // 256 * 256
        if self.arena is None or self.arena.device != device or self.used + nbytes > self.arena.numel():
            size = max(2 * nbytes, 64 << 20, 0 if self.arena is None else 2 * self.arena.numel())
            if self.arena is not None:
                self.pending = self.pending + (self.arena,)
            self.arena, self.used = torch.empty(size, dtype=torch.uint8, device=device), 0
        piece = self.arena[self.used:self.used + nbytes]
        self.used += nbytes
        pin(self.arena)
        return piece

    def release(self):
        self.used, self.pending = 0, ()


_ws = Workspace()

import os as _os

_SIDE = {'streams': [], 'ws': [Workspace()], 'n': max(1, int(_os.environ.get('NIMG_SIDE_STREAMS', '2'))), 'next': 0, 'keys': {},
         'enabled': _os.environ.get('NIMG_NO_SIDE_STREAM') is None, 'dirty': set()}
_ws_side = _SIDE['ws'][0]


def _side_index(key):
    if key is None or _SIDE['n'] == 1:
        return 0
    k = _SIDE['keys'].get(key)
    if k is None:
        k = _SIDE['keys'][key] = _SIDE['next'] % _SIDE['n']
        _SIDE['next'] += 1
    return k


_TICKETS = {}
TICKETS = _os.environ.get('NIMG_TICKETS') is not None


def _bind_tickets(device, handle):
    key = (device.index, handle)
    buf = _TICKETS.get(key)
    if buf is None:
        buf = _TICKETS[key] = torch.zeros(_lib.TICKET_BYTES, dtype=torch.uint8, device=device)
        _lib.call('nimg_bind_tickets', handle, buf.data_ptr(), buf.numel())
    pin(buf)


def _ws_current(device):
    cur = _stream() if (_raw_device is not None and device.index in (None, _raw_device())) else \
        torch.cuda.current_stream(device).cuda_stream
    if TICKETS:
        _bind_tickets(device, cur)
    for k, st in enumerate(_SIDE['streams']):
        if st is not None and st.device == device and cur == st.cuda_stream:
            return _SIDE['ws'][k]
    return _ws


SIDE_CUS = int(_os.environ.get('NIMG_SIDE_CUS', '0'))


def _new_side_stream(dev):
    if SIDE_CUS <= 0:
        return torch.cuda.Stream(device=dev)
    import ctypes
    h = ctypes.c_void_p()
    with torch.cuda.device(dev):
        _lib.call('nimg_stream_create_cu_mask', SIDE_CUS, ctypes.byref(h))
    return torch.cuda.ExternalStream(h.value, device=dev)


class _on_side_stream(object):
    def __init__(self, *tensors, key=None):
        self.tensors = [t for t in tensors if t is not None]
        self.k = _side_index(key)

    def __enter__(self):
        dev = self.tensors[0].device
        streams, k = _SIDE['streams'], self.k
        while len(streams) <= k:
            streams.append(None)
            if len(_SIDE['ws']) < len(streams):
                _SIDE['ws'].append(Workspace())
        if streams[k] is None or streams[k].device != dev:
            streams[k] = _new_side_stream(dev)
        side = streams[k]
        self.prev = torch.cuda.current_stream(dev)
        fork = _SIDE.get('fork')
        if fork is not None and fork[1] == self.prev:
            if k not in fork[2]:
                side.wait_event(fork[0])
                fork[2].add(k)
        else:
            side.wait_stream(self.prev)
        for t in self.tensors:
            t.record_stream(side)
        torch.cuda.set_stream(side)
        _SIDE['dirty'].add(k)
        return side

    def __exit__(self, *exc):
        torch.cuda.set_stream(self.prev)
        return False


FORK_GROUPS = _os.environ.get('NIMG_NO_FORK_GROUPS') is None


class one_fork(object):
    def __enter__(self):
        if FORK_GROUPS and _SIDE['enabled'] and _SIDE.get('fork') is None and torch.cuda.is_available():
            cur = torch.cuda.current_stream()
            ev = torch.cuda.Event()
            ev.record(cur)
            _SIDE['fork'] = (ev, cur, set())
            self.mine = True
        else:
            self.mine = False
        return self

    def __exit__(self, *exc):
        if self.mine:
            _SIDE['fork'] = None
        return False


class ParamGroup(object):

    def __init__(self, defer=True):
        self.fns = []
        self.defer = defer

    def add(self, fn):
        if self.defer and FORK_GROUPS and _SIDE['enabled']:
            self.fns.append(fn)
        else:
            fn()

    def flush(self):
        if self.fns:
            with one_fork():
                for fn in self.fns:
                    fn()
            self.fns = []


class side_stream(object):

    def __init__(self, *tensors, key=None):
        self.ctx = _on_side_stream(*tensors, key=key) if _SIDE['enabled'] else None

    def __enter__(self):
        return self.ctx.__enter__() if self.ctx is not None else None

    def __exit__(self, *exc):
        return self.ctx.__exit__(*exc) if self.ctx is not None else False


DEFER_REDUCE = _os.environ.get('NIMG_DEFER_REDUCE') is not None
_DEFER = {}


def _defer_state(k):
    st = _DEFER.get(k)
    if st is None:
        import ctypes
        lib = _lib.load()
        nb, cap = int(lib.nimg_reduce_entry_bytes()), int(lib.nimg_reduce_batch_max())
        st = _DEFER[k] = {'buf': (ctypes.c_char * (nb * cap))(), 'n': 0, 'nb': nb, 'cap': cap}
    return st


def _flush_deferred(k, on_its_stream=True):
    st = _DEFER.get(k)
    if st is None or st['n'] == 0:
        return
    side = _SIDE['streams'][k]
    if on_its_stream and side is not None and torch.cuda.current_stream(side.device) != side:
        prev = torch.cuda.current_stream(side.device)
        torch.cuda.set_stream(side)
        try:
            _lib.call('nimg_reduce_slabs_batch', st['buf'], st['n'], _stream())
        finally:
            torch.cuda.set_stream(prev)
    else:
        _lib.call('nimg_reduce_slabs_batch', st['buf'], st['n'], _stream())
    st['n'] = 0
    _SIDE['ws'][k].release()


CHAIN_REDUCE = _os.environ.get('NIMG_CHAIN_REDUCE', '0') == '1'
_CHAIN = {}
REDUCE_STREAM = _os.environ.get('NIMG_REDUCE_STREAM', '0') == '1'
_RSTREAM = {'streams': {}, 'dirty': set()}


def _reduce_carrier():
    if DEFER_REDUCE:
        return 'defer'
    if REDUCE_STREAM:
        return 'stream'
    if CHAIN_REDUCE:
        return 'chain'
    return None


def _reduce_behind(k, entry, device):
    side = torch.cuda.current_stream(device)
    rs = _RSTREAM['streams'].get(k)
    if rs is None or rs.device != device:
        rs = _RSTREAM['streams'][k] = torch.cuda.Stream(device=device)
    ev = torch.cuda.Event()
    ev.record(side)
    rs.wait_event(ev)
    torch.cuda.set_stream(rs)
    try:
        _lib.call('nimg_reduce_slabs_batch', entry, 1, _stream())
    finally:
        torch.cuda.set_stream(side)
    _RSTREAM['dirty'].add(k)


def _flush_chain(k):
    entry = _CHAIN.pop(k, None)
    if entry is None:
        return
    side = _SIDE['streams'][k]
    prev = torch.cuda.current_stream(side.device)
    torch.cuda.set_stream(side)
    try:
        _lib.call('nimg_reduce_slabs_batch', entry, 1, _stream())
    finally:
        torch.cuda.set_stream(prev)
    _SIDE['ws'][k].release()


def join_side_stream():
    for k in sorted(_SIDE['dirty']):
        st = _SIDE['streams'][k]
        if st is not None:
            _flush_deferred(k)
            _flush_chain(k)
            torch.cuda.current_stream(st.device).wait_stream(st)
    _SIDE['dirty'].clear()
    for k in sorted(_RSTREAM['dirty']):
        rs = _RSTREAM['streams'][k]
        torch.cuda.current_stream(rs.device).wait_stream(rs)
        _SIDE['ws'][k].release()
    _RSTREAM['dirty'].clear()


def qtable(quality, channel):
    out = np.zeros(64, np.float32)
    _lib.call('nimg_jpeg_qtable', int(quality), int(channel), out.ctypes.data)
    return out.reshape(8, 8)


def qtables_device(quality, device):
    q = np.stack([qtable(quality, 0), qtable(quality, 1), qtable(quality, 1)]) if quality is not None \
        else np.ones((3, 8, 8), np.float32)
    return torch.from_numpy(q).to(device)


ROUNDING = {'round': 0, 'soft': 1, 'sin': 2, 'harmonic': 3, 'identity': 4}


def djpeg_fwd(x, qtab, rounding='soft', want_mask=True, want_idx=False, want_xdq=False, out=None):
    _f32(x, qtab, out)
    n, h, w, c = x.shape
    if c != 3:
        raise ValueError('dJPEG expects NHW3 images')
    y = torch.empty_like(x) if out is None else out
    mask = torch.empty((n, h, w), dtype=torch.uint8, device=x.device) if want_mask else None
    idx = torch.empty((n, 3, h // 8, w // 8, 8, 8), dtype=torch.int16, device=x.device) if want_idx else None
    xdq = torch.empty((n, 3, h // 8, w // 8, 8, 8), dtype=torch.float32, device=x.device) if want_xdq else None
    _lib.call('nimg_djpeg_fwd', _p(x), _p(y), _p(qtab), _p(mask), _p(idx), _p(xdq), n, h, w, ROUNDING[rounding],
              _stream())
    return y, mask, idx, xdq


def djpeg_bwd(x, gy, mask, qtab, rounding='soft', out=None, dq=None, accumulate=False):
    _f32(x, gy, qtab, dq)
    _chk(mask)
    n, h, w, _ = x.shape
    gx = torch.empty_like(x) if out is None else out
    if dq is None:
        _lib.call('nimg_djpeg_bwd', _p(x), _p(gy), _p(mask), _p(qtab), _p(gx), n, h, w, ROUNDING[rounding], _stream())
        return gx
    if dq.numel() != 128 or not dq.is_contiguous():
        raise ValueError('dq: 128 contiguous float32 values (2 x 8 x 8) expected')
    need = _lib.load().nimg_djpeg_dq_workspace_bytes(n, h, w)
    ws = _ws_current(x.device).get(need, x.device)
    _lib.call('nimg_djpeg_bwd_dq', _p(x), _p(gy), _p(mask), _p(qtab), _p(gx), _p(dq), n, h, w, ROUNDING[rounding],
              1 if accumulate else 0, _p(ws), need, _stream())
    return gx


def _djpeg_sub_shape(x, hs, vs):
    if x.dim() != 4 or x.shape[3] != 3:
        raise ValueError('dJPEG expects NHW3 images')
    if (hs, vs) not in ((2, 1), (2, 2)):
        raise ValueError('sub-sampled dJPEG: sampling factors (2,1) or (2,2) expected, got ({},{}) - 4:4:4 is djpeg_fwd / '
                         'djpeg_bwd'.format(hs, vs))
    n, h, w, _ = x.shape
    if h <= 0 or w <= 0 or h % (8 * vs) or w % (8 * hs):
        raise ValueError('sub-sampled dJPEG needs whole MCUs: h % {} == 0 and w % {} == 0, got {} x {}'.format(8 * vs, 8 * hs, h, w))
    return n, h, w


def _djpeg_sub_views(buf, n, h, w, hs, vs):
    hb, wb, hcb, wcb = h // 8, w // 8, h // (8 * vs), w // (8 * hs)
    return buf[:, :hb * wb * 64].view(n, hb, wb, 8, 8), buf[:, hb * wb * 64:].view(n, 2, hcb, wcb, 8, 8)


def djpeg_sub_fwd(x, qtab, rounding='soft', hs=2, vs=2, want_mask=True, want_idx=False, want_xdq=False, out=None):
    _f32(x, qtab, out)
    n, h, w = _djpeg_sub_shape(x, hs, vs)
    y = torch.empty_like(x) if out is None else out
    mask = torch.empty((n, h, w), dtype=torch.uint8, device=x.device) if want_mask else None
    per_image = (h // 8 * (w // 8) + 2 * (h // (8 * vs)) * (w // (8 * hs))) * 64
    idx = torch.empty((n, per_image), dtype=torch.int16, device=x.device) if want_idx else None
    xdq = torch.empty((n, per_image), dtype=torch.float32, device=x.device) if want_xdq else None
    need = _lib.load().nimg_djpeg_sub_workspace_bytes(n, h, w, hs, vs, 0)
    ws = _ws_current(x.device).get(need, x.device)
    _lib.call('nimg_djpeg_sub_fwd', _p(x), _p(y), _p(qtab), _p(mask), _p(idx), _p(xdq), n, h, w, hs, vs, ROUNDING[rounding],
              _p(ws), need, _stream())
    return (y, mask, _djpeg_sub_views(idx, n, h, w, hs, vs) if want_idx else None,
            _djpeg_sub_views(xdq, n, h, w, hs, vs) if want_xdq else None)


def djpeg_sub_bwd(x, gy, mask, qtab, rounding='soft', hs=2, vs=2, out=None, dq=None, accumulate=False):
    _f32(x, gy, qtab, dq)
    _chk(mask)
    n, h, w = _djpeg_sub_shape(x, hs, vs)
    gx = torch.empty_like(x) if out is None else out
    if dq is not None and (dq.numel() != 128 or not dq.is_contiguous()):
        raise ValueError('dq: 128 contiguous float32 values (2 x 8 x 8) expected')
    need = _lib.load().nimg_djpeg_sub_workspace_bytes(n, h, w, hs, vs, 0 if dq is None else 1)
    ws = _ws_current(x.device).get(need, x.device)
    _lib.call('nimg_djpeg_sub_bwd', _p(x), _p(gy), _p(mask), _p(qtab), _p(gx), _p(dq), n, h, w, hs, vs, ROUNDING[rounding],
              1 if accumulate else 0, _p(ws), need, _stream())
    return gx


def conv2d(x, w, bias=None, x2=None, stride=1, padding='SAME', act=None, pad_mode=0, out=None, out2=None,
           act_mask=None, pads=None, out_hw=None, _wmode=0, _f32_only=False, mask_alpha=None, out_bf16=False, residual=None,
           bf16_copy=False, d2s_out=False, s2d_out=False, copy_lrelu=False, mask_conv_layout=False):
    copy = None
    if mask_conv_layout and not d2s_out:
        raise ValueError('mask_conv_layout only has a meaning with d2s_out')
    if w.shape[0] not in (1, 2, 3, 5):
        if w.shape[0] not in BIG_KERNELS or stride != 1:
            raise NotImplementedError('convolution kernel size {} (stride {}) is not built: 1 ... 11 at stride 1'.format(
                w.shape[0], stride))
        _f32_only = True
    if s2d_out:
        co_ = w.shape[3] if _wmode == 0 else w.shape[2]
        fused = COMPUTE == 'bf16' and not _f32_only and x2 is None and out is None and out2 is None and stride == 1 and \
            w.shape[0] == 3 and co_ % 4 == 0 and co_ >= 8 and x.shape[3] % 4 == 0 and x.shape[3] >= 8 and \
            (x.shape[3] % 8 == 0 or (not _is_bf16(x) and residual is None)) and D2S_EPILOGUE and not bf16_copy and \
            not d2s_out
        if not fused:
            y = conv2d(x, w, bias, stride=stride, padding=padding, act=act, pad_mode=pad_mode, act_mask=act_mask, pads=pads,
                       out_hw=out_hw, _wmode=_wmode, _f32_only=_f32_only, mask_alpha=mask_alpha, residual=residual)
            y = d2s_clip_bwd(y, 1.0)
            return y.to(torch.bfloat16) if out_bf16 and COMPUTE == 'bf16' else y
    if d2s_out:
        co_ = w.shape[3] if _wmode == 0 else w.shape[2]
        fused = COMPUTE == 'bf16' and not _f32_only and x2 is None and out is None and out2 is None and stride == 1 and \
            w.shape[0] == 3 and co_ % 16 == 0 and x.shape[3] % 8 == 0 and D2S_EPILOGUE
        if residual is not None:
            raise NotImplementedError('d2s_out with a residual')
        if not fused:
            if mask_conv_layout:
                raise RuntimeError('a space-to-depth-stored mask needs the fused depth-to-space epilogue')
            y = conv2d(x, w, bias, stride=stride, padding=padding, act=act, pad_mode=pad_mode, pads=pads, out_hw=out_hw,
                       _wmode=_wmode, _f32_only=_f32_only)
            y = d2s_clip(y, 1.0, 0.0, False)
            y = y if act_mask is None else lrelu_bwd(y, act_mask, out=y, alpha=mask_alpha)
            if out_bf16 and COMPUTE == 'bf16':
                y = y.to(torch.bfloat16)
            return (y, y.to(torch.bfloat16) if COMPUTE == 'bf16' else None) if bf16_copy else y
    if residual is not None or bf16_copy:
        _f32(residual)
        fused = COMPUTE == 'bf16' and not _f32_only and x2 is None and out2 is None and \
            ((stride == 1 and w.shape[0] == 3) or (residual is None and (w.shape[0], stride) in ((1, 1), (5, 1), (5, 2)))) and \
            (s2d_out or (not out_bf16 and (out is None or out.dtype == torch.float32))) and x.shape[3] % 8 == 0 and \
            not (copy_lrelu and act is not None) and \
            (w.shape[3] if _wmode == 0 else w.shape[2]) % 4 == 0 and (w.shape[3] if _wmode == 0 else w.shape[2]) >= 8
        if not fused:
            y = conv2d(x, w, bias, x2=x2, stride=stride, padding=padding, act=act, pad_mode=pad_mode, out=out, out2=out2,
                       act_mask=act_mask, pads=pads, out_hw=out_hw, _wmode=_wmode, _f32_only=_f32_only, mask_alpha=mask_alpha,
                       out_bf16=out_bf16)
            if residual is not None:
                add(residual, y, out=y)
            return (y, None) if bf16_copy else y
    _f32(w, bias)
    _fb(x, x2, out, out2, act_mask)
    if (x2 is not None and x2.dtype != x.dtype) or (out2 is not None and out is not None and out2.dtype != out.dtype):
        raise RuntimeError('the two halves of a split input / output must be stored alike (both float32 or both bfloat16)')
    n, h, wd, c1 = x.shape
    c2 = 0 if x2 is None else x2.shape[3]
    ks = w.shape[0]
    cout = w.shape[3] if _wmode == 0 else w.shape[2]
    if (w.shape[2] if _wmode == 0 else w.shape[3]) != c1 + c2 or w.shape[1] != ks:
        raise ValueError('weight shape {} does not match input channels {}+{}'.format(tuple(w.shape), c1, c2))
    if pads is not None:
        pt, pl = pads
        ho, wo = out_hw
    elif padding == 'SAME':
        ho, pt = same_pads(h, ks, stride)
        wo, pl = same_pads(wd, ks, stride)
    elif padding == 'VALID':
        pt = pl = 0
        ho, wo = (h - ks) // stride + 1, (wd - ks) // stride + 1
    else:
        raise ValueError(padding)
    if s2d_out and (ho % 2 or wo % 2):
        raise ValueError('s2d_out: even output size expected')
    if out is None:
        shape = (n, 2 * ho, 2 * wo, cout // 4) if d2s_out else ((n, ho // 2, wo // 2, 4 * cout) if s2d_out else (n, ho, wo, cout))
        out = torch.empty(shape, dtype=torch.bfloat16 if out_bf16 else torch.float32, device=x.device)
    o1 = cout if (d2s_out or s2d_out) else out.shape[3]
    o2 = 0 if out2 is None else out2.shape[3]
    if o1 + o2 != cout or (not (d2s_out or s2d_out) and tuple(out.shape[:3]) != (n, ho, wo)):
        raise ValueError('output shape mismatch')
    if d2s_out and act_mask is not None and \
            tuple(act_mask.shape) != ((n, ho, wo, cout) if mask_conv_layout else tuple(out.shape)):
        raise ValueError('d2s_out: the mask has the shape of the depth-to-space output (or of the convolution, mask_conv_layout)')
    if act not in (None, 'leaky_relu', 'relu'):
        raise ValueError('unsupported activation {}'.format(act))
    act_id = 0 if act is None else 1
    alpha = 0.0 if act == 'relu' else (LRELU_ALPHA if mask_alpha is None else float(mask_alpha))
    if COMPUTE == 'bf16' and not _f32_only and _wmode == 0 and c2 == 0 and out2 is None and act_mask is None and \
            c1 in (3, 4) and ks in (3, 5) and stride == 1 and cout >= 8 and (ho, wo) == (h, wd) and \
            (pt, pl) == ((ks - 1) // 2, (ks - 1) // 2):
        _f32(x)
        if ROWS_CONV and c1 == 4 and ks == 3 and cout == 32 and wd == 128 and h % 4 == 0 and h >= 4 and pad_mode == 0 and \
                _is_bf16(out) and act in (None, 'leaky_relu') and n * h * wd * 16 < (1 << 31) - 65536:
            _lib.call('nimg_conv3_rows_c4_bf16', _p(x), _p(w), _p(bias), _p(out), n, h, wd, act_id, alpha, _stream())
            return out
        _lib.call('nimg_conv2d_fwd_smallc_bf16_ex', _p(x), c1, _p(w), _p(bias), _p(out), cout, n, h, wd, ks, pad_mode,
                  act_id, alpha, BF16_OUT if _is_bf16(out) else 0, _stream())
        return out
    if COMPUTE == 'bf16' and not _f32_only and _wmode == 1 and c2 == 0 and out2 is None and act_mask is None and \
            c1 == 32 and cout == 3 and ks == 5 and stride == 1 and (ho, wo) == (h, wd) and (pt, pl) == (2, 2) and \
            pad_mode == 0 and bias is None and act is None and not _is_bf16(x) and not _is_bf16(out):
        _lib.call('nimg_conv2d_dgrad_fewin_bf16', _p(x), _p(w), _p(out), 3, 32, n, h, wd, 5, _stream())
        return out
    if COMPUTE == 'bf16' and not _f32_only and residual is None and not bf16_copy and not d2s_out and not s2d_out and \
            rows_conv_ok(x, x2, ks, stride, cout, (ho, wo), (pt, pl), pad_mode, out, out2, act_mask, act, bias):
        _lib.call('nimg_conv3_rows_bf16', _p(x), c1, _p(x2), c2, _p(weights_bf16(w, _wmode)), _p(bias), _p(act_mask), _p(out),
                  _p(out2), None, n, h, wd, cout, act_id, alpha, 0 if _is_bf16(out) else 1, _stream())
        return out if out2 is None else (out, out2)
    if COMPUTE == 'bf16' and not _f32_only and c2 % 8 == 0 and cout >= 8 and \
            (c1 % 8 == 0 or (c2 == 0 and c1 % 4 == 0 and c1 >= 8 and not _is_bf16(x))):
        wb = weights_bf16(w, _wmode)
        flags = (BF16_IN if _is_bf16(x) else 0) | (BF16_OUT if _is_bf16(out) else 0) | \
            (BF16_MASK if _is_bf16(act_mask) else 0) | (D2S_OUT if d2s_out else 0) | (S2D_OUT if s2d_out else 0) | \
            (MASK_CONV if (mask_conv_layout and d2s_out) else 0)
        if residual is not None or bf16_copy:
            if residual is not None and tuple(residual.shape) != (n, ho, wo, cout):
                raise ValueError('residual: the shape of the output expected')
            if bf16_copy:
                copy = torch.empty(out.shape, dtype=torch.bfloat16, device=out.device)
            _lib.call('nimg_conv2d_fwd_bf16_res', _p(x), c1, _p(wb), _p(bias), _p(out), o1, _p(act_mask), _p(residual), _p(copy),
                      n, h, wd, ks, stride, pt, pl, pad_mode, ho, wo, act_id, alpha, flags | (COPY_LRELU if copy_lrelu else 0),
                      _stream())
            return (out, copy) if bf16_copy else out
        _lib.call('nimg_conv2d_fwd_bf16_ex', _p(x), c1, _p(x2), c2, _p(wb), _p(bias), _p(out), o1, _p(out2), o2,
                  _p(act_mask), n, h, wd, ks, stride, pt, pl, pad_mode, ho, wo, act_id, alpha, flags, _stream())
        return out if out2 is None else (out, out2)
    if _is_bf16(x) or _is_bf16(out) or _is_bf16(act_mask) or _is_bf16(x2) or _is_bf16(out2):
        raise RuntimeError('bf16-stored tensor reached a float32 convolution path')
    if _wmode == 1:
        w = flip_weights(w)
    _lib.call('nimg_conv2d_fwd', _p(x), c1, _p(x2), c2, _p(w), _p(bias), _p(out), o1, _p(out2), o2, _p(act_mask),
              n, h, wd, ks, stride, pt, pl, pad_mode, ho, wo, act_id, alpha, _stream())
    return out if out2 is None else (out, out2)


ROWS_CONV = _os.environ.get('NIMG_NO_ROWS_CONV') is None
ROWS_LEVEL2 = _os.environ.get('NIMG_ROWS_LEVEL2') is not None


def rows_conv_ok(x, x2, ks, stride, cout, out_hw, pads, pad_mode, out, out2, act_mask, act, bias=None):
    n, h, wd, c1 = x.shape
    c2 = 0 if x2 is None else x2.shape[3]
    if ROWS_CONV and ROWS_LEVEL2 and ks == 3 and stride == 1 and wd == 64 and h % 4 == 0 and h >= 4 and tuple(out_hw) == (h, wd) and \
            tuple(pads) == (1, 1) and pad_mode == 0 and _is_bf16(x) and x2 is None and act in (None, 'leaky_relu') and \
            n * h * wd * max(c1, 64) * 2 < (1 << 31) - 65536:
        return cout == 64 and c1 in (32, 64) and out2 is None and _is_bf16(out) and out.shape[3] == 64 and \
            (act_mask is None or (_is_bf16(act_mask) and tuple(act_mask.shape) == (n, h, wd, 64)))
    if not (ROWS_CONV and ks == 3 and stride == 1 and wd == 128 and h % 4 == 0 and h >= 4 and tuple(out_hw) == (h, wd) and
            tuple(pads) == (1, 1) and pad_mode == 0 and _is_bf16(x) and (x2 is None or _is_bf16(x2)) and
            act in (None, 'leaky_relu') and n * h * wd * max(c1, c2) * 2 < (1 << 31) - 65536):
        return False
    if cout == 64:
        return (c1, c2) == (32, 0) and out2 is not None and _is_bf16(out) and _is_bf16(out2) and out.shape[3] == 32 and \
            out2.shape[3] == 32 and act_mask is None and bias is None and act is None
    return cout == 32 and out2 is None and (c1, c2) in ((32, 0), (64, 0), (32, 32)) and \
        (act_mask is None or (_is_bf16(act_mask) and tuple(act_mask.shape) == (n, h, wd, 32)))


def rows_d2s_ok(x, w):
    n, h, wd, c = x.shape
    return ROWS_CONV and COMPUTE == 'bf16' and _is_bf16(x) and tuple(w.shape) == (3, 3, 32, 12) and c == 32 and wd == 128 and \
        h % 4 == 0 and h >= 4 and n * h * wd * 64 < (1 << 31) - 65536


def conv3_rows_d2s(x, w, bias, out=None):
    if not rows_d2s_ok(x, w):
        raise ValueError('conv3_rows_d2s: unsupported shape / mode')
    _f32(w, bias, out)
    n, h, wd, _ = x.shape
    if out is not None and (tuple(out.shape) != (n, 2 * h, 2 * wd, 3) or not out.is_contiguous()):
        raise ValueError('conv3_rows_d2s: output shape mismatch')
    y = torch.empty((n, 2 * h, 2 * wd, 3), dtype=torch.float32, device=x.device) if out is None else out
    _lib.call('nimg_conv3_rows_d2s_bf16', _p(x), 32, _p(weights_bf16(w, 0)), _p(bias), _p(y), n, h, wd, _stream())
    return y


def flip_weights(w, out=None):
    _f32(w, out)
    kh, kw, cin, cout = w.shape
    wt = torch.empty((kh, kw, cout, cin), dtype=torch.float32, device=w.device) if out is None else out
    _lib.call('nimg_conv_flip_weights', _p(w), _p(wt), kh, kw, cin, cout, _stream())
    return wt


def conv2d_dgrad(dz, w, in_hw, stride=1, padding='SAME', act_mask=None, out=None, out2=None, mask_alpha=None,
                 out_bf16=False, residual=None, bf16_copy=False, d2s_out=False, s2d_out=False, mask_conv_layout=False):
    if stride != 1:
        raise NotImplementedError('strided dgrad is expressed by the caller (see models/compression.py)')
    ks = w.shape[0]
    h, wd = in_hw
    if padding == 'SAME':
        _, pt = same_pads(h, ks, 1)
        _, pl = same_pads(wd, ks, 1)
    else:
        pt = pl = 0
    return conv2d(dz, w, None, pads=(ks - 1 - pt, ks - 1 - pl), out_hw=(h, wd), act_mask=act_mask, out=out,
                  out2=out2, _wmode=1, mask_alpha=mask_alpha, out_bf16=out_bf16, residual=residual, bf16_copy=bf16_copy,
                  d2s_out=d2s_out, s2d_out=s2d_out, mask_conv_layout=mask_conv_layout)


def conv2d_wgrad(x, dz, ks, x2=None, stride=1, padding='SAME', pad_mode=0, pads=None, dw=None, accumulate=False,
                 db=None, side=False, _defer_k=None):
    if side and _SIDE['enabled'] and dw is not None:
        ctx = _on_side_stream(x, dz, x2, key=dw.data_ptr())
        with ctx:
            return conv2d_wgrad(x, dz, ks, x2=x2, stride=stride, padding=padding, pad_mode=pad_mode, pads=pads, dw=dw,
                                accumulate=accumulate, db=db, side=False, _defer_k=ctx.k)
    _f32(dw, db)
    _fb(x, x2, dz)
    if x2 is not None and x2.dtype != x.dtype:
        raise RuntimeError('the two halves of a split input must be stored alike (both float32 or both bfloat16)')
    n, h, wd, c1 = x.shape
    c2 = 0 if x2 is None else x2.shape[3]
    _, ho, wo, cout = dz.shape
    if pads is not None:
        pt, pl = pads
    elif padding == 'SAME':
        _, pt = same_pads(h, ks, stride)
        _, pl = same_pads(wd, ks, stride)
    else:
        pt = pl = 0
    if dw is None:
        dw = torch.empty((ks, ks, c1 + c2, cout), dtype=torch.float32, device=x.device)
    packed_ok = c2 == 0 and c1 in (3, 4) and stride == 1 and ks in (3, 5)
    if ks not in (1, 2, 3, 5) and (ks not in BIG_KERNELS or stride != 1):
        raise NotImplementedError('weight gradient for kernel size {} (stride {}) is not built'.format(ks, stride))
    if COMPUTE == 'bf16' and ks in (1, 2, 3, 5) and (packed_ok or (c1 % 4 == 0 and c2 % 4 == 0 and cout % 4 == 0 and c1 + c2 >= 8 and
                                            (c2 == 0 or c1 % 8 == 0))):
        need = _lib.load().nimg_conv2d_wgrad_bf16_workspace_bytes(c1 + c2, cout, ks, ks, n, ho, wo)
        flags = (BF16_IN if _is_bf16(x) else 0) | (BF16_DZ if _is_bf16(dz) else 0)
        carrier = _reduce_carrier() if _defer_k is not None and not accumulate else None
        if carrier:
            _wgrad_carried(_defer_k, carrier, x.device, need, flags, _p(x), c1, _p(x2), c2, _p(dz), None, cout, _p(dw), _p(db), n, h, wd,
                           ks, stride, pt, pl, pad_mode, ho, wo)
            return dw
        if _defer_k is not None and CHAIN_REDUCE:
            _flush_chain_here(_defer_k)
        if _defer_k is not None:
            _flush_deferred(_defer_k, on_its_stream=False)
        ws = _ws_current(x.device).get(need, x.device)
        _lib.call('nimg_conv2d_wgrad_bf16_ex', _p(x), c1, _p(x2), c2, _p(dz), cout, _p(dw), _p(db), n, h, wd, ks, stride,
                  pt, pl, pad_mode, ho, wo, 1 if accumulate else 0, _p(ws), ws.numel(), flags, _stream())
        return dw
    if _is_bf16(x) or _is_bf16(dz):
        raise RuntimeError('bf16-stored tensor reached a float32 weight-gradient path')
    need = _lib.load().nimg_conv2d_wgrad_workspace_bytes(c1 + c2, cout, ks, ks, n, ho, wo)
    ws = _ws_current(x.device).get(need, x.device)
    _lib.call('nimg_conv2d_wgrad', _p(x), c1, _p(x2), c2, _p(dz), cout, _p(dw), _p(db), n, h, wd, ks, stride, pt, pl,
              pad_mode, ho, wo, 1 if accumulate else 0, _p(ws), ws.numel(), _stream())
    return dw


# ... 1581 lines not shown
```

### neural-imaging_amd/workflows/manipulation_classification.py

```python
from collections import OrderedDict

import os

import numpy as np
import torch

from .. import ops, parallel
from ..device import DeviceArray, to_device
from ..helpers import tf_helpers
from ..models import forensics, jpeg, pipelines


class ManipulationClassification(object):

    def __init__(self, nip_model, manipulations=None, distribution=None, fan_args=None, trainable=None,
                 raw_patch_size=128, loss_metric='L2', device=None, nan_check='eager', pipeline_fan_update=None):
        if raw_patch_size < 16 or raw_patch_size > 512:
            raise ValueError('The patch size ({}) looks incorrect, typical values should be >= 16 and <= 512'.format(
                raw_patch_size))
        self._trainable = set() if trainable is None else set(trainable)
        self._trainable.add('fan')
        if distribution is None:
            self._distribution = {'downsampling': 'pool:2', 'compression': 'jpeg',
                                  'compression_params': {'quality': 50, 'codec': 'soft'}}
        else:
            self._distribution = dict(distribution)
        if ':' in nip_model:
            nip_model, nip_pretrained_dirname = nip_model.split(':')
        else:
            nip_pretrained_dirname = None
        if not hasattr(pipelines, nip_model) or not isinstance(getattr(pipelines, nip_model), type) or \
                not issubclass(getattr(pipelines, nip_model), pipelines.NIPModel):
            raise ValueError('Invalid NIP model ({})! Available NIPs: ({})'.format(nip_model, pipelines.supported_models))
        if loss_metric not in ['L2', 'L1', 'SSIM']:
            raise ValueError('Invalid loss metric ({})!'.format(loss_metric))

        self.nip = getattr(pipelines, nip_model)(loss_metric=loss_metric, patch_size=raw_patch_size, device=device)
        self.device = self.nip.device
        if nip_pretrained_dirname is not None:
            self.nip.load_model(nip_pretrained_dirname)

        manipulations = manipulations or ['sharpen', 'resample', 'gaussian', 'jpeg']
        self._strengths = {'sharpen': 1, 'resample': 50, 'gaussian': 0.83, 'jpeg': 80, 'awgn': 5.1, 'gamma': 3,
                           'median': 3}
        self._strengths_range = {'sharpen': (0.25, 1.5), 'resample': (40, 90), 'gaussian': (0.5, 7),
                                 'jpeg': (50, 90), 'awgn': (1, 5), 'gamma': (1, 5), 'median': (3, 9)}
        manipulations_set = set()
        for m in manipulations:
            spec = m.split(':')
            manipulations_set.add(spec[0])
            if len(spec) > 1:
                self._strengths[spec[0]] = float(spec[-1])
        if any(x not in self._strengths.keys() for x in manipulations_set):
            raise ValueError('Unsupported manipulation requested! Available: {}'.format(self._strengths.keys()))

        self._jpeg_manip = jpeg.JPEG(None, 'soft', device=self.device)
        self._operations = OrderedDict()
        self._forensics_classes = ['native']
        builders = OrderedDict([('sharpen', tf_helpers.Sharpen), ('resample', tf_helpers.Resample),
                                ('gaussian', tf_helpers.Gaussian), ('jpeg', None), ('awgn', tf_helpers.Awgn),
                                ('gamma', tf_helpers.Gamma), ('median', tf_helpers.Median)])
        for name, cls in builders.items():
            if name not in manipulations_set:
                continue
            if name == 'jpeg':
                self._operations[name] = _JpegManipulation(self._jpeg_manip)
            elif cls is None:
                raise NotImplementedError('manipulation {} is not built yet'.format(name))
            else:
                self._operations[name] = cls()
            self._forensics_classes.append('{}:{}'.format(name, self._strengths[name]))
        assert len(self._forensics_classes) == self.n_classes

        if self._distribution['compression'] == 'jpeg':
            self.codec = jpeg.JPEG(device=self.device, **self._distribution['compression_params'])
        elif self._distribution['compression'] == 'dcn':
            from ..models import compression
            params = self._distribution['compression_params']
            self.codec = params['model'] if 'model' in params else compression.TwitterDCN.restore(
                params['dirname'], device=self.device)
            self._distribution = dict(self._distribution, compression_params={
                k: v for k, v in params.items() if k != 'model'})
        elif self._distribution['compression'] == 'none':
            self.codec = None
        else:
            raise ValueError('Unsupported channel compression {}'.format(self._distribution['compression']))
        if 'dcn' in self._trainable and (self.codec is None or len(self.codec.parameters) == 0):
            raise ValueError('The current codec does not appear to be trainable: {}!'.format(
                None if self.codec is None else self.codec.class_name))

        self._is_dcn = self._distribution['compression'] == 'dcn'
        fan_input_patch = 2 * raw_patch_size // self.downsampling_factor
        self.fan = forensics.FAN(n_classes=self.n_classes, patch_size=fan_input_patch, device=self.device,
                                 **(fan_args or {}))
        self._parameters = list(self.fan.parameters)
        if 'nip' in self._trainable:
            self._parameters.extend(self.nip.parameters)
        if 'dcn' in self._trainable:
            self._parameters.extend(self.codec.parameters)
        self._step = 0
        self._nan_check = nan_check
        self._nan_flag = torch.zeros(1, dtype=torch.int32, device=self.device)
        self._nan_seen = torch.zeros(1, dtype=torch.int32, device=self.device)
        self._labels_cache = {}
        self._lr_t_dev = None
        self._bucket = parallel.GradientBucket()
        if pipeline_fan_update is None:
            pipeline_fan_update = os.environ.get('NIMG_PIPELINE_FAN', '0') == '1'
        self._pipeline_fan = bool(pipeline_fan_update)
        self._pending_fan = None

    @property
    def n_classes(self):
        return len(self._operations) + 1

    @property
    def downsampling_factor(self):
        if self._distribution['downsampling'] == 'none':
            return 1
        elif ':' in self._distribution['downsampling']:
            return int(self._distribution['downsampling'].split(':')[-1])
        return 2

    def _batch_labels(self, batch_size):
        return np.concatenate([x * np.ones((batch_size,), dtype=np.int32) for x in range(self.n_classes)])

    def _device_labels(self, batch_size):
        if batch_size not in self._labels_cache:
            self._labels_cache[batch_size] = torch.from_numpy(self._batch_labels(batch_size)).to(self.device)
        return self._labels_cache[batch_size]

    def _manipulations(self, Y, randomize=False, override=None, training=False, m=None):
        override = override if override is not None else self._strengths
        b = Y.shape[0]
        if m is None:
            m = torch.empty((self.n_classes * b,) + tuple(Y.shape[1:]), dtype=torch.float32, device=Y.device)
            m[:b].copy_(Y)
        elif Y.data_ptr() != m.data_ptr() or m.shape[0] != self.n_classes * b:
            raise ValueError('the class batch must start with the developed images')
        ctxs = []
        names = list(self._operations.keys())
        if randomize:
            drawn = parallel.broadcast_floats([np.random.uniform(*self._strengths_range[n]) for n in names], Y.device)
            strengths = dict(zip(names, drawn))
        else:
            strengths = override
        for k, (name, op) in enumerate(self._operations.items()):
            s = strengths[name]
            _, ctx = op.forward(Y, s, out=m[(k + 1) * b:(k + 2) * b], training=training)
            ctxs.append(ctx)
        return m, ctxs

    def _downsampling(self, m):
        factor = self.downsampling_factor
        mode = self._distribution['downsampling']
        if mode.startswith('pool'):
            return ops.avgpool(m, factor)
        elif mode == 'bilinear':
            op = self._bilinear_operator(m.shape[1], factor, m.device)
            tmp = ops.sparse_axis_apply(m, op.fwd, 0, op.out_size)
            return ops.sparse_axis_apply(tmp, op.fwd, 1, op.out_size)
        elif mode == 'none':
            return m
        raise ValueError('Unsupported channel down-sampling {}'.format(mode))

    def _bilinear_operator(self, size, factor, device):
        from ..helpers import kernels as hk
        key = (size, factor, str(device))
        cache = self.__dict__.setdefault('_bilinear_cache', {})
        if key not in cache:
            cache[key] = ops.AxisOperator(hk.bilinear_axis_matrix(size, size // factor), device)
        return cache[key]

    def _downsampling_bwd(self, dc):
        mode = self._distribution['downsampling']
        if mode.startswith('pool'):
            return ops.avgpool_bwd(dc, self.downsampling_factor)
        if mode == 'bilinear':
            op = self._bilinear_operator(dc.shape[1] * self.downsampling_factor, self.downsampling_factor, dc.device)
            tmp = ops.sparse_axis_apply(dc, op.bwd, 0, op.in_size)
            return ops.sparse_axis_apply(tmp, op.bwd, 1, op.in_size)
        return dc

    def run_workflow(self, batch_x, augment=False, training=False):
        self.finish_pending()
        x = to_device(batch_x, self.device)
        Y = self.nip.forward(x)[0]
        m, _ = self._manipulations(Y, augment)
        c = self._downsampling(m)
        C, ent, _ = self._codec_forward(c)
        entropy = np.nan if ent is None else DeviceArray(ent)
        probs = self.fan.forward(C)[0]
        return DeviceArray(Y), DeviceArray(c), DeviceArray(C), entropy, DeviceArray(probs)

    def run_workflow_to_decisions(self, batch_x):
        return self.run_workflow(batch_x)[-1].numpy().argmax(axis=1)

    def run_manipulations(self, batch_y, randomize=False, override=None):
        return DeviceArray(self._manipulations(to_device(batch_y, self.device), randomize, override)[0])

    def manipulations_timing(self, batch_y):
        from datetime import datetime
        Y = to_device(batch_y, self.device)
        times = {}
        for name, op in self._operations.items():
            torch.cuda.synchronize(self.device)
            d1 = datetime.now()
            op.forward(Y, self._strengths[name])
            torch.cuda.synchronize(self.device)
            times[name] = (datetime.now() - d1).total_seconds()
        return times

    def run_downsampling(self, batch_y):
        return DeviceArray(self._downsampling(to_device(batch_y, self.device)))

    def run_compression(self, batch_y, return_entropy=False):
        y = to_device(batch_y, self.device)
        C, ent, _ = self._codec_forward(y)
        return (DeviceArray(C), np.nan if ent is None else DeviceArray(ent)) if return_entropy else DeviceArray(C)

    def run_rgb_to_fan(self, batch_Y):
        m = self._manipulations(to_device(batch_Y, self.device))[0]
        c = self._downsampling(m)
        return self._codec_forward(c)[0].cpu().numpy()

    def run_rgb_to_probabilities(self, batch_Y):
        self.finish_pending()
        C = torch.from_numpy(self.run_rgb_to_fan(batch_Y)).to(self.device)
        return self.fan.forward(C)[0].cpu().numpy()

    def _codec_forward(self, c, training=False):
        if self.codec is None:
            return c, None, None
        if self._is_dcn:
            return self.codec.forward(c, training=training)
        C, ctx = self.codec.forward(c, training=training)
        return C, None, ctx

    def training_step(self, batch_x, batch_y, lambda_nip=0, lambda_dcn=0, augment=False, learning_rate=1e-4):
        x = to_device(batch_x, self.device)
        target = to_device(batch_y, self.device)
        b = x.shape[0]
        train_nip = 'nip' in self._trainable and self.nip.count_parameters() > 0
        train_dcn = 'dcn' in self._trainable
        need_upstream = train_nip or train_dcn
        world = parallel.world_size()

        self._launch_pending_fan()

        m = None
        if getattr(self.nip, 'writes_into', False):
            b = x.shape[0]
            m = torch.empty((self.n_classes * b, 2 * x.shape[1], 2 * x.shape[2], 3), dtype=torch.float32, device=x.device)
            Y, nctx = self.nip.forward(x, training=train_nip, out=m[:b])
        else:
            Y, nctx = self.nip.forward(x, training=train_nip)
        m, mctxs = self._manipulations(Y, augment, training=train_nip, m=m)
        c = self._downsampling(m)
        C, entropy, cctx = self._codec_forward(c, training=need_upstream)
        self._finish_pending_fan()
        _, fctx = self.fan.forward(C, self._device_labels(b), training=True)

        ops.int_fill(self._nan_flag, 0)
        late_fan = forensics.LATE_PARAMS and need_upstream and not parallel.is_distributed() and \
            C.shape[0] >= forensics.LATE_MIN_IMAGES
        pipelined = self._pipeline_fan and need_upstream and not parallel.is_distributed() and self._nan_check == 'deferred' and \
            self._lr_t_dev is None
        deferred = [] if pipelined else None
        if pipelined:
            late_fan = True
        loss_ce, dC = self.fan.backward(fctx, need_input_grad=need_upstream, join=not late_fan, defer=deferred)
        if not late_fan:
            ops.nan_flag(self.fan._model.flat_grad, self._nan_flag)
            self._bucket.launch(self.fan._model.flat_grad)
        loss_dcn = None
        dc = None
        if need_upstream:
            if self.codec is None:
                dc = dC
            elif self._is_dcn:
                lam = float(lambda_dcn) * world if train_dcn else 0.0
                dc_direct = None
                if train_dcn:
                    l2, _ = ops.l2_loss(c, C, grad_scale=lam, grad_out=dC, accumulate=True)
                    if train_nip:
                        dc_direct = torch.empty_like(c)
                        ops.l2_loss(C, c, grad_scale=lam, grad_out=dc_direct, accumulate=False)
                    loss_dcn = (l2, entropy)
                dc = self.codec.backward(cctx, dC, entropy_coef=lam * self.codec._h.entropy_weight,
                                         need_input_grad=train_nip)
                if train_nip and dc_direct is not None:
                    ops.add(dc, dc_direct, out=dc)
                if train_dcn:
                    ops.nan_flag(self.codec._model.flat_grad, self._nan_flag)
                    self._bucket.launch(self.codec._model.flat_grad)
            else:
                dc_direct = None
                if train_dcn:
                    lam = float(lambda_dcn) / (255.0 * 255.0)
                    mse, _ = ops.mse255(C, c, grad_scale=lam, grad_out=dC, accumulate=True)
                    if train_nip:
                        dc_direct = torch.empty_like(c)
                        ops.mse255(c, C, grad_scale=lam, grad_out=dc_direct, accumulate=False)
                    loss_dcn = (mse, None)
                dc = self.codec.backward(cctx, dC)
                if dc_direct is not None:
                    ops.add(dc, dc_direct, out=dc)
                if train_dcn:
                    ops.nan_flag(self.codec._model.flat_grad, self._nan_flag)
                    self._bucket.launch(self.codec._model.flat_grad)
        if train_nip:
            dm = self._downsampling_bwd(dc)
            parts_dY = [dm[:b]] + [op.backward(mctxs[k], dm[(k + 1) * b:(k + 2) * b])
                                   for k, (name, op) in enumerate(self._operations.items())]
            dY = dm[:b]
            head = self.nip.head_gradient(parts_dY, Y, target, float(lambda_nip)) if hasattr(self.nip, 'head_gradient') else None
            nip_kw = {}
            if head is not None:
                loss_nip, nip_kw['dz_head'] = head
            else:
                for i in range(0, len(parts_dY) - 1, 5):
                    chunk = ([dY] if i else [parts_dY[0]]) + parts_dY[i + 1:i + 6]
                    ops.add_n(chunk, out=dY)
                loss_nip, _ = self.nip.loss_and_grad(Y, target, grad_scale=float(lambda_nip), grad_out=dY, accumulate=True)
            if parallel.is_distributed() and hasattr(self.nip, 'decoder_grads'):
                dec, enc = self.nip.decoder_grads()
                def decoder_done():
                    ops.nan_flag(dec, self._nan_flag)
                    self._bucket.launch(dec)
                self.nip.backward(nctx, dY, on_decoder_done=decoder_done, **nip_kw)
                ops.nan_flag(enc, self._nan_flag)
                self._bucket.launch(enc)
            else:
                self.nip.backward(nctx, dY, **nip_kw)
                ops.nan_flag(self.nip._model.flat_grad, self._nan_flag)
                self._bucket.launch(self.nip._model.flat_grad)
        else:
            loss_nip, _ = self.nip._loss_fn(Y, target)
        if late_fan and not pipelined:
            ops.nan_flag(self.fan._model.flat_grad, self._nan_flag)
            self._bucket.launch(self.fan._model.flat_grad)
        parallel.all_reduce_flag(self._nan_flag)
        ops.int_max_(self._nan_seen, self._nan_flag)
        if self._nan_check == 'eager' and int(self._nan_flag.item()) != 0:
            self._nan_seen.zero_()
            self._bucket.wait()
            raise RuntimeError('gradient NaNs in the workflow step')
        self._bucket.wait()

        self._step += 1
        gscale = 1.0 / world
        rate = self._lr_t_dev
        if pipelined:
            self._pending_fan = (deferred, learning_rate, self._step, gscale)
        else:
            self.fan._model.adam(learning_rate, self._step, gscale, skip_flag=self._nan_flag, lr_t_dev=rate)
        if train_nip:
            self.nip._model.adam(learning_rate, self._step, gscale, skip_flag=self._nan_flag, lr_t_dev=rate)
        if train_dcn:
            self.codec._model.adam(learning_rate, self._step, gscale, skip_flag=self._nan_flag, lr_t_dev=rate)

        dcn_value = np.nan
        if loss_dcn is not None and loss_dcn[1] is None:
            dcn_value = _LazySum(torch.zeros_like(loss_dcn[0]), loss_dcn[0], 1.0 / (255.0 * 255.0))
        elif loss_dcn is not None:
            dcn_value = _LazySum(loss_dcn[0], loss_dcn[1], self.codec._h.entropy_weight)
        loss = _LazyLoss(loss_ce, loss_nip, float(lambda_nip) if 'nip' in self._trainable else 0.0,
                         dcn_value if loss_dcn is not None else None, float(lambda_dcn))
        return loss, {'ce': DeviceArray(loss_ce), 'nip': DeviceArray(loss_nip), 'dcn': dcn_value}

    def _launch_pending_fan(self):
        if self._pending_fan is not None and self._pending_fan[0] is not None:
            with ops.one_fork():
                for fn in self._pending_fan[0]:
                    fn()
            self._pending_fan = (None,) + self._pending_fan[1:]

    def _finish_pending_fan(self):
        if self._pending_fan is None:
            return
        self._launch_pending_fan()
        _, lr, step, gscale = self._pending_fan
        self._pending_fan = None
        ops.nan_flag(self.fan._model.flat_grad, self._nan_flag)
        ops.int_max_(self._nan_seen, self._nan_flag)
        self.fan._model.adam(lr, step, gscale, skip_flag=self._nan_flag)

    def finish_pending(self):
        self._finish_pending_fan()

    def check_nan(self):
        self.finish_pending()
        """Deferred NaN guard (nan_check='deferred'): raises if any step since the last check produced NaN grads (those
        steps' Adam updates were skipped on the device)."""
        seen = int(self._nan_seen.item())
        self._nan_seen.zero_()
        if seen != 0:
            raise RuntimeError('gradient NaNs in the workflow step')

    def summary_compact(self):
        return '{class_name}[{trainables}]: {nip} -> [{manips}] {pool}{codec}-> {fan}'.format(
            class_name=type(self).__name__, nip=self.nip.class_name,
            manips=''.join([x[0] for x in self._forensics_classes]),
            trainables=''.join([x[0] for x in self.trainable_models]),
            pool='' if self._distribution['downsampling'] == 'none' else '-> {} '.format(
                self._distribution['downsampling']),
            codec='' if self.codec is None else '-> {} '.format(self.codec.summary_compact()), fan='FAN')

    def summary(self):
        return '{class_name}[opt={trainables}]: {input} -> {nip} -> {n_ops} manipulations [{manips}] {pool}{codec}-> {fan}'.format(
            class_name=type(self).__name__, input='(rgb)' if self.nip.x.shape[-1] == 3 else '(raw)',
            nip=self.nip.class_name, n_ops=self.n_classes - 1,
            manips=''.join([x[0] for x in self._forensics_classes]),
            trainables=''.join([x[0] for x in self.trainable_models]),
            pool='' if self._distribution['downsampling'] == 'none' else '-> {} '.format(
                self._distribution['downsampling']),
            codec='' if self.codec is None else '-> {} '.format(self.codec.summary_compact()),
            fan='FAN -> (prob. {} classes)'.format(self.n_classes))

    def details(self):
        out = [self.summary()]
        out.append('Input         : {} {}'.format(self.nip.x.shape, '(rgb)' if self.nip.x.shape[-1] == 3 else '(raw)'))
        out.append('Camera ISP    : {}'.format(self.nip.summary()))
        out.append('Manipulations : {} -> {}'.format(self.n_classes, self._forensics_classes))
        out.append('Downsampling  : {}'.format(self._distribution['downsampling']))
        out.append('Codec         : {}'.format('' if self.codec is None else self.codec.summary()))
        out.append('Forensics     : {}'.format(self.fan.summary()))
        out.append('Output        : {}'.format(self.fan.y.shape))
        return '\n'.join(out)

    def is_trainable(self, model):
        return model in self._trainable

    @property
    def trainable_models(self):
        return tuple(x for x in self._trainable)


class _JpegManipulation(object):

    def __init__(self, codec):
        self.codec = codec

    def forward(self, x, quality, out=None, training=False):
        return self.codec.forward(x, quality, training=training, out=out)

    def backward(self, ctx, dy):
        return self.codec.backward(ctx, dy)


class _LazySum(DeviceArray):
    __slots__ = ('a', 'b', 'w')

    def __init__(self, a, b, w):
        self.t = a
        self.a, self.b, self.w = a, b, float(w)

    def numpy(self):
        return np.asarray(float(self.a.detach().cpu().reshape(())) + self.w * float(self.b.detach().cpu().reshape(())))

    def __float__(self):
        return float(self.numpy())


class _LazyLoss(DeviceArray):
    __slots__ = ('ce', 'nip', 'lam', 'dcn', 'lam_dcn')

    def __init__(self, ce, nip, lam, dcn=None, lam_dcn=0.0):
        self.t = ce
        self.ce, self.nip, self.lam, self.dcn, self.lam_dcn = ce, nip, lam, dcn, lam_dcn

    def numpy(self):
        v = self.ce.detach().cpu().numpy().reshape(()) + np.float32(self.lam) * self.nip.detach().cpu().numpy().reshape(())
        extra = 0.0 if self.dcn is None else self.lam_dcn * float(self.dcn)
        return np.asarray(v + np.float32(extra), dtype=np.float32)

    def __float__(self):
        return float(self.numpy())
```

Before: 8464 patches/s.

## Fuse JPEG manipulation and JPEG channel codec into single chained kernels

Adds chained dJPEG forward and backward kernels. The JPEG manipulation branch is compressed twice (manipulation QF then channel QF) inside one kernel without a round-trip through global memory, and the plain branches get channel compression in the same launch. The workflow defers the jpeg manipulation and routes it plus the codec through these kernels when the configuration qualifies. This removes separate launches and the intermediate image writes and reads, in exchange for a more complex code path and a bespoke backward that reproduces the two quantisation masks.

```diff
diff --git a/include/nimg.h b/include/nimg.h
--- a/include/nimg.h
+++ b/include/nimg.h
@@ -42,6 +42,13 @@
 int nimg_djpeg_bwd_dq(const float* x, const float* gy, const uint8_t* mask, const float* qtab, float* gx, float* dq,
                       int n, int h, int w, int rounding, int accumulate, void* workspace, size_t workspace_bytes,
                       void* stream);
+int nimg_djpeg_chain_fwd(const float* x_plain, const float* y_src, float* t_out , float* C, const float* q1,
+                         const float* q2, uint8_t* mask1 , uint8_t* mask2 , int n_plain,
+                         int n_comp, int h, int w, int rounding1, int rounding2, int shared, void* stream);
+int nimg_djpeg_chain_bwd(const float* x_plain, const float* y_src, const float* t_src , const float* gC,
+                         const uint8_t* mask1, const uint8_t* mask2, const float* q1, const float* q2, float* g_plain,
+                         float* g_comp, int n_plain, int n_comp, int h, int w, int rounding1, int rounding2, int shared,
+                         void* stream);
 size_t nimg_djpeg_sub_workspace_bytes(int n, int h, int w, int hs, int vs, int with_dq);
 int nimg_djpeg_sub_fwd(const float* x, float* y, const float* qtab, uint8_t* mask, int16_t* idx, float* xdq,
                        int n, int h, int w, int hs, int vs, int rounding, void* workspace, size_t workspace_bytes,
diff --git a/neural-imaging_amd/_lib.py b/neural-imaging_amd/_lib.py
--- a/neural-imaging_amd/_lib.py
+++ b/neural-imaging_amd/_lib.py
@@ -11,6 +11,8 @@
     'nimg_abi_version': (c_int, []),
     'nimg_djpeg_fwd': (c_int, [P, P, P, P, P, P, c_int, c_int, c_int, c_int, P]),
     'nimg_djpeg_bwd': (c_int, [P, P, P, P, P, c_int, c_int, c_int, c_int, P]),
+    'nimg_djpeg_chain_fwd': (c_int, [P, P, P, P, P, P, P, P, c_int, c_int, c_int, c_int, c_int, c_int, c_int, P]),
+    'nimg_djpeg_chain_bwd': (c_int, [P, P, P, P, P, P, P, P, P, P, c_int, c_int, c_int, c_int, c_int, c_int, c_int, P]),
     'nimg_djpeg_dq_workspace_bytes': (c_size_t, [c_int, c_int, c_int]),
     'nimg_djpeg_bwd_dq': (c_int, [P, P, P, P, P, P, c_int, c_int, c_int, c_int, c_int, P, c_size_t, P]),
     'nimg_djpeg_sub_workspace_bytes': (c_size_t, [c_int, c_int, c_int, c_int, c_int, c_int]),
diff --git a/neural-imaging_amd/csrc/djpeg.h b/neural-imaging_amd/csrc/djpeg.h
--- a/neural-imaging_amd/csrc/djpeg.h
+++ b/neural-imaging_amd/csrc/djpeg.h
@@ -188,6 +188,27 @@
     __syncthreads();
     return __builtin_amdgcn_readfirstlane(*flag) != 0;
 }
+__device__ __forceinline__ void stage_tables_pair(const float* __restrict__ qa, const float* __restrict__ qb, float* qTa,
+                                                  float* qTb, bool& fast_a, bool& fast_b) {
+    const int tid = threadIdx.x;
+    int* fa = reinterpret_cast<int*>(qTa + 384);
+    int* fb = reinterpret_cast<int*>(qTb + 384);
+    if (tid == 0) { *fa = 1; *fb = 1; }
+    __syncthreads();
+    if (tid < 192) {
+        const float a = qa[tid], bq = qb[tid];
+        const int c = tid >> 6, u = (tid >> 3) & 7, r = tid & 7;
+        qTa[(c * 8 + r) * 8 + u] = a;
+        qTa[192 + (c * 8 + r) * 8 + u] = 1.0f / a;
+        qTb[(c * 8 + r) * 8 + u] = bq;
+        qTb[192 + (c * 8 + r) * 8 + u] = 1.0f / bq;
+        if (!(a >= 1.0f && a <= 255.0f && a == rintf(a))) *fa = 0;
+        if (!(bq >= 1.0f && bq <= 255.0f && bq == rintf(bq))) *fb = 0;
+    }
+    __syncthreads();
+    fast_a = __builtin_amdgcn_readfirstlane(*fa) != 0;
+    fast_b = __builtin_amdgcn_readfirstlane(*fb) != 0;
+}
 __device__ __forceinline__ void read_tables(const float* qT, int c, int r, float (&q)[8], float (&rc)[8]) {
 #pragma unroll
     for (int k = 0; k < 2; ++k) {
diff --git a/neural-imaging_amd/csrc/djpeg.hip b/neural-imaging_amd/csrc/djpeg.hip
--- a/neural-imaging_amd/csrc/djpeg.hip
+++ b/neural-imaging_amd/csrc/djpeg.hip
@@ -8,6 +8,7 @@
 constexpr int TILE_F = 3 * 8 * 72;
 constexpr int WAVE_LDS_F = (STAGE_F > TILE_F ? STAGE_F : TILE_F);
 constexpr int WAVES_PER_BLOCK = 4;
+constexpr int TABLES_F = 384 + 4;
 #ifndef DJ_FWD_WGS
 #define DJ_FWD_WGS 4
 #endif
@@ -37,6 +38,58 @@
         }
         dct_inv8(X, v[c]);
     }
+}
+
+template <int QMODE>
+__device__ __forceinline__ void codec_rows(float* lds, const float* qT, bool fast, bool active, const Task& t, int b, int r,
+                                           int hb, int wb, int16_t* __restrict__ idx, float* __restrict__ xdq,
+                                           float (&px)[24], uint32_t& mlo, uint32_t& mhi) {
+    constexpr float kRc255 = 1.0f / 255.0f;
+    float v[3][8];
+    {
+        float ycc[3][8];
+        colour_fwd(px, ycc);
+#pragma unroll
+        for (int c = 0; c < 3; ++c) dct_fwd8(ycc[c], v[c]);
+    }
+    transpose24(lds, b, r, v);
+    if (active) {
+        if (fast) quantise_columns<QMODE, false>(v, qT, t, b, r, hb, wb, idx, xdq);
+        else quantise_columns<QMODE, true>(v, qT, t, b, r, hb, wb, idx, xdq);
+    }
+    transpose24(lds, b, r, v);
+    float q3[3][8];
+#pragma unroll
+    for (int c = 0; c < 3; ++c) {
+        dct_inv8(v[c], q3[c]);
+#pragma unroll
+        for (int j = 0; j < 8; ++j) q3[c][j] += 127.0f;
+    }
+    mlo = 0;
+    mhi = 0;
+#pragma unroll
+    for (int j = 0; j < 8; ++j) {
+        uint32_t m = 0;
+#pragma unroll
+        for (int c = 0; c < 3; ++c) {
+            float acc = kCI[c][0];
+            acc = __builtin_fmaf(q3[0][j], kCI[c][1], acc);
+            acc = __builtin_fmaf(q3[1][j], kCI[c][2], acc);
+            acc = __builtin_fmaf(q3[2][j], kCI[c][3], acc);
+            acc = div_q<false>(acc, 255.0f, kRc255);
+            const float cl = __builtin_amdgcn_fmed3f(acc, 0.0f, 1.0f);
+            m |= cl == acc ? (1u << c) : 0u;
+            px[3 * j + c] = cl;
+        }
+        if (j < 4) mlo |= m << (8 * j); else mhi |= m << (8 * (j - 4));
+    }
+}
+
+__device__ __forceinline__ uint2* mask_row(uint8_t* mask, const Task& t, int h, int w, int b, int r) {
+    return reinterpret_cast<uint2*>(mask + ((long)t.n * h + t.by * 8 + r) * w + t.x0 + b * 8);
+}
+__device__ __forceinline__ const uint2* mask_row(const uint8_t* mask, const Task& t, int h, int w, int b, int r) {
+    return reinterpret_cast<const uint2*>(mask + ((long)t.n * h + t.by * 8 + r) * w + t.x0 + b * 8);
 }
 
 template <int QMODE>
@@ -53,7 +106,6 @@
     const long n_tasks = (long)n * hb * strips;
     const Task t = decode_task((long)blockIdx.x * WAVES_PER_BLOCK + wave, n_tasks, hb, strips);
     const bool active = t.valid && (t.x0 + b * 8 < w);
-    constexpr float kRc255 = 1.0f / 255.0f;
 
     f32x4 pre[6] = {};
     fetch_strip(x, pre, t, h, w, lane);
@@ -61,52 +113,129 @@
     commit_strip(lds, pre, lane);
     wave_sync();
     float px[24];
-    float v[3][8];
     read_row24(lds, b, r, px);
     wave_sync();
-    {
-        float ycc[3][8];
-        colour_fwd(px, ycc);
-#pragma unroll
-        for (int c = 0; c < 3; ++c) dct_fwd8(ycc[c], v[c]);
-    }
-    transpose24(lds, b, r, v);
+    uint32_t mlo, mhi;
+    codec_rows<QMODE>(lds, qT, fast, active, t, b, r, hb, wb, idx, xdq, px, mlo, mhi);
+    write_row24(lds, b, r, px);
+    if (mask && active) *mask_row(mask, t, h, w, b, r) = make_uint2(mlo, mhi);
+    wave_sync();
+    store_strip(y, lds, t, h, w, lane);
+}
+
+template <int QMODE2>
+__global__ __launch_bounds__(256, DJ_FWD_WGS) void djpeg_chain_fwd_kernel(
+    const float* __restrict__ x_plain, const float* __restrict__ y_src, float* __restrict__ t_out, float* __restrict__ C,
+    const float* __restrict__ q1, const float* __restrict__ q2, uint8_t* __restrict__ mask1, uint8_t* __restrict__ mask2,
+    int n_plain, int n_comp, int first_plain, int shared, int h, int w) {
+    extern __shared__ __attribute__((aligned(16))) float smem[];
+    const int wave = threadIdx.x >> 6, lane = threadIdx.x & 63;
+    const int b = lane >> 3, r = lane & 7;
+    float* lds = smem + wave * WAVE_LDS_F;
+    float* qT1 = smem + WAVES_PER_BLOCK * WAVE_LDS_F;
+    float* qT2 = qT1 + TABLES_F;
+    const int hb = h / 8, wb = w / 8, strips = (w + STRIP_PX - 1) / STRIP_PX;
+    const long n_tasks = (long)(n_comp + n_plain - first_plain) * hb * strips;
+    Task t = decode_task((long)blockIdx.x * WAVES_PER_BLOCK + wave, n_tasks, hb, strips);
+    const bool comp = __builtin_amdgcn_readfirstlane((int)(t.valid && t.n < n_comp)) != 0;
+    if (!comp && t.valid) t.n += first_plain - n_comp;
+    const bool active = t.valid && (t.x0 + b * 8 < w);
+
+    f32x4 pre[6] = {};
+    fetch_strip(comp ? y_src : x_plain, pre, t, h, w, lane);
+    bool fast1, fast2;
+    stage_tables_pair(q1, q2, qT1, qT2, fast1, fast2);
+    commit_strip(lds, pre, lane);
+    wave_sync();
+    float px[24];
+    read_row24(lds, b, r, px);
+    wave_sync();
+    uint32_t mlo, mhi;
+    if (comp) {
+        codec_rows<Q_RINT>(lds, qT1, fast1, active, t, b, r, hb, wb, nullptr, nullptr, px, mlo, mhi);
+        if (t_out || shared) {
+            write_row24(lds, b, r, px);
+            wave_sync();
+            if (t_out) store_strip(t_out, lds, t, h, w, lane);
+            if (shared) store_strip(C, lds, t, h, w, lane);
+            wave_sync();
+        }
+        if (active) {
+            if (mask1) *mask_row(mask1, t, h, w, b, r) = make_uint2(mlo, mhi);
+            if (shared && mask2) *mask_row(mask2, t, h, w, b, r) = make_uint2(mlo, mhi);
+        }
+        t.n += n_plain;
+    }
+    codec_rows<QMODE2>(lds, qT2, fast2, active, t, b, r, hb, wb, nullptr, nullptr, px, mlo, mhi);
+    write_row24(lds, b, r, px);
+    if (mask2 && active) *mask_row(mask2, t, h, w, b, r) = make_uint2(mlo, mhi);
+    wave_sync();
+    store_strip(C, lds, t, h, w, lane);
+}
+
+__device__ __forceinline__ void grad_rows_x(const float (&px)[24], float (&tx)[3][8]) {
+    float ycc[3][8];
+    colour_fwd(px, ycc);
+#pragma unroll
+    for (int c = 0; c < 3; ++c) dct_fwd8(ycc[c], tx[c]);
+}
+#define DJ_GRAD_ROWS_G(px, mm, tg)                                                                                        \
+    {                                                                                                                     \
+        _Pragma("clang fp contract(fast)")                                                                                \
+        float gq[3][8];                                                                                                   \
+        _Pragma("unroll")                                                                                                 \
+        for (int j = 0; j < 8; ++j) {                                                                                     \
+            const uint32_t m = ((j < 4 ? mm.x >> (8 * j) : mm.y >> (8 * (j - 4)))) & 0xffu;                               \
+            float g[3];                                                                                                   \
+            _Pragma("unroll")                                                                                             \
+            for (int c = 0; c < 3; ++c) g[c] = (m >> c) & 1u ? px[3 * j + c] * (1.0f / 255.0f) : 0.0f;                    \
+            _Pragma("unroll")                                                                                             \
+            for (int c = 0; c < 3; ++c)                                         \
+                gq[c][j] = g[0] * kCI[0][1 + c] + g[1] * kCI[1][1 + c] + g[2] * kCI[2][1 + c];                            \
+        }                                                                                                                 \
+        _Pragma("unroll")                                                                                                 \
+        for (int c = 0; c < 3; ++c) dct_fwd8(gq[c], tg[c]);                                                               \
+    }
+#define DJ_GRAD_ROWS_OUT(tg, px, lds, b, r)                                                                               \
+    {                                                                                                                     \
+        _Pragma("clang fp contract(fast)")                                                                                \
+        float gb[3][8];                                                                                                   \
+        _Pragma("unroll")                                                                                                 \
+        for (int c = 0; c < 3; ++c) dct_inv8(tg[c], gb[c]);                                                 \
+        _Pragma("unroll")                                                                                                 \
+        for (int j = 0; j < 8; ++j)                                                                                       \
+            _Pragma("unroll")                                                                                             \
+            for (int c = 0; c < 3; ++c)                                \
+                px[3 * j + c] =                                                                                           \
+                    255.0f * (gb[0][j] * kCF[0][1 + c] + gb[1][j] * kCF[1][1 + c] + gb[2][j] * kCF[2][1 + c]);            \
+        write_row24(lds, b, r, px);                                                                                       \
+    }
+template <int GMODE, int QMODE, bool DQ, int ND>
+__device__ __forceinline__ void grad_columns(float* lds, const float* qT, bool fast, bool active, int b, int r,
+                                             float (&tx)[3][8], float (&tg)[3][8], float (&dqa)[ND][8]) {
+    transpose24(lds, b, r, tx);
+    transpose24(lds, b, r, tg);
     if (active) {
-        if (fast) quantise_columns<QMODE, false>(v, qT, t, b, r, hb, wb, idx, xdq);
-        else quantise_columns<QMODE, true>(v, qT, t, b, r, hb, wb, idx, xdq);
-    }
-    transpose24(lds, b, r, v);
-    {
-        float q3[3][8];
-#pragma unroll
-        for (int c = 0; c < 3; ++c) {
-            dct_inv8(v[c], q3[c]);
-#pragma unroll
-            for (int j = 0; j < 8; ++j) q3[c][j] += 127.0f;
-        }
-        uint32_t mlo = 0, mhi = 0;
-#pragma unroll
-        for (int j = 0; j < 8; ++j) {
-            uint32_t m = 0;
+        auto columns = [&](auto exact) {
 #pragma unroll
             for (int c = 0; c < 3; ++c) {
-                float acc = kCI[c][0];
-                acc = __builtin_fmaf(q3[0][j], kCI[c][1], acc);
-                acc = __builtin_fmaf(q3[1][j], kCI[c][2], acc);
-                acc = __builtin_fmaf(q3[2][j], kCI[c][3], acc);
-                acc = div_q<false>(acc, 255.0f, kRc255);
-                const float cl = __builtin_amdgcn_fmed3f(acc, 0.0f, 1.0f);
-                m |= cl == acc ? (1u << c) : 0u;
-                px[3 * j + c] = cl;
+                float X[8], G[8], q[8], rc[8];
+                dct_fwd8(tx[c], X);
+                dct_fwd8(tg[c], G);
+                read_tables(qT, c, r, q, rc);
+#pragma unroll
+                for (int u = 0; u < 8; ++u) {
+                    const float z = div_q<decltype(exact)::value>(X[u], q[u], rc[u]);
+                    const float qg = quantise_grad<GMODE>(z);
+                    if constexpr (DQ) dqa[c == 0 ? 0 : 1][u] += G[u] * (quantise<QMODE>(z) - z * qg);
+                    G[u] *= qg;
+                }
+                dct_inv8(G, tg[c]);
             }
-            if (j < 4) mlo |= m << (8 * j); else mhi |= m << (8 * (j - 4));
-        }
-        write_row24(lds, b, r, px);
-        if (mask && active)
-            *reinterpret_cast<uint2*>(mask + ((long)t.n * h + t.by * 8 + r) * w + t.x0 + b * 8) = make_uint2(mlo, mhi);
-    }
-    wave_sync();
-    store_strip(y, lds, t, h, w, lane);
+        };
+        if (fast) columns(std::false_type{});
+        else columns(std::true_type{});
+    }
 }
 
 template <int RND, bool DQ>
@@ -134,38 +263,16 @@
     commit_strip(lds, pre, lane);
     fetch_strip(gy, pre, t, h, w, lane);
     uint2 mm = make_uint2(0u, 0u);
-    if (active) mm = *reinterpret_cast<const uint2*>(mask + ((long)t.n * h + t.by * 8 + r) * w + t.x0 + b * 8);
+    if (active) mm = *mask_row(mask, t, h, w, b, r);
     wave_sync();
     read_row24(lds, b, r, px);
     wave_sync();
-    {
-        float ycc[3][8];
-        colour_fwd(px, ycc);
-#pragma unroll
-        for (int c = 0; c < 3; ++c) dct_fwd8(ycc[c], tx[c]);
-    }
+    grad_rows_x(px, tx);
     commit_strip(lds, pre, lane);
     wave_sync();
     read_row24(lds, b, r, px);
     wave_sync();
-    {
-#pragma clang fp contract(fast)
-        float gq[3][8];
-#pragma unroll
-        for (int j = 0; j < 8; ++j) {
-            const uint32_t m = ((j < 4 ? mm.x >> (8 * j) : mm.y >> (8 * (j - 4)))) & 0xffu;
-            float g[3];
-#pragma unroll
-            for (int c = 0; c < 3; ++c) g[c] = (m >> c) & 1u ? px[3 * j + c] * (1.0f / 255.0f) : 0.0f;
-#pragma unroll
-            for (int c = 0; c < 3; ++c)
-                gq[c][j] = g[0] * kCI[0][1 + c] + g[1] * kCI[1][1 + c] + g[2] * kCI[2][1 + c];
-        }
-#pragma unroll
-        for (int c = 0; c < 3; ++c) dct_fwd8(gq[c], tg[c]);
-    }
-    transpose24(lds, b, r, tx);
-    transpose24(lds, b, r, tg);
+    DJ_GRAD_ROWS_G(px, mm, tg)
     float dqa[DQ ? 2 : 1][8];
     if constexpr (DQ) {
 #pragma unroll
@@ -173,27 +280,7 @@
 #pragma unroll
             for (int u = 0; u < 8; ++u) dqa[k][u] = 0.0f;
     }
-    if (active) {
-        auto columns = [&](auto exact) {
-#pragma unroll
-            for (int c = 0; c < 3; ++c) {
-                float X[8], G[8], q[8], rc[8];
-                dct_fwd8(tx[c], X);
-                dct_fwd8(tg[c], G);
-                read_tables(qT, c, r, q, rc);
-#pragma unroll
-                for (int u = 0; u < 8; ++u) {
-                    const float z = div_q<decltype(exact)::value>(X[u], q[u], rc[u]);
-                    const float qg = quantise_grad<GMODE>(z);
-                    if constexpr (DQ) dqa[c == 0 ? 0 : 1][u] += G[u] * (quantise<QMODE>(z) - z * qg);
-                    G[u] *= qg;
-                }
-                dct_inv8(G, tg[c]);
-            }
-        };
-        if (fast) columns(std::false_type{});
-        else columns(std::true_type{});
-    }
+    grad_columns<GMODE, QMODE, DQ>(lds, qT, fast, active, b, r, tx, tg, dqa);
     if constexpr (DQ) {
         const long task = (long)blockIdx.x * WAVES_PER_BLOCK + wave;
 #pragma unroll
@@ -208,25 +295,94 @@
             }
     }
     transpose24(lds, b, r, tg);
-    {
-#pragma clang fp contract(fast)
-        float gb[3][8];
-#pragma unroll
-        for (int c = 0; c < 3; ++c) dct_inv8(tg[c], gb[c]);
-#pragma unroll
-        for (int j = 0; j < 8; ++j)
-#pragma unroll
-            for (int c = 0; c < 3; ++c)
-                px[3 * j + c] =
-                    255.0f * (gb[0][j] * kCF[0][1 + c] + gb[1][j] * kCF[1][1 + c] + gb[2][j] * kCF[2][1 + c]);
-        write_row24(lds, b, r, px);
-    }
+    DJ_GRAD_ROWS_OUT(tg, px, lds, b, r)
     wave_sync();
     store_strip(gx, lds, t, h, w, lane);
 }
 
+template <int RND2>
+__global__ __launch_bounds__(256, DJ_BWD_WGS) void djpeg_chain_bwd_kernel(
+    const float* __restrict__ x_plain, const float* __restrict__ y_src, const float* __restrict__ t_src,
+    const float* __restrict__ gC, const uint8_t* __restrict__ mask1, const uint8_t* __restrict__ mask2,
+    const float* __restrict__ q1, const float* __restrict__ q2, float* __restrict__ g_plain, float* __restrict__ g_comp,
+    int n_plain, int n_comp, int h, int w) {
+    constexpr int GMODE2 = bwd_mode(RND2), QMODE2 = fwd_mode(RND2);
+    extern __shared__ __attribute__((aligned(16))) float smem[];
+    const int wave = threadIdx.x >> 6, lane = threadIdx.x & 63;
+    const int b = lane >> 3, r = lane & 7;
+    float* lds = smem + wave * WAVE_LDS_F;
+    float* qT1 = smem + WAVES_PER_BLOCK * WAVE_LDS_F;
+    float* qT2 = qT1 + TABLES_F;
+    const int hb = h / 8, wb = w / 8, strips = (w + STRIP_PX - 1) / STRIP_PX;
+    const long n_tasks = (long)(n_comp + n_plain) * hb * strips;
+    Task t = decode_task((long)blockIdx.x * WAVES_PER_BLOCK + wave, n_tasks, hb, strips);
+    const bool comp = __builtin_amdgcn_readfirstlane((int)(t.valid && t.n < n_comp)) != 0;
+    if (!comp && t.valid) t.n -= n_comp;
+    Task tc = t;
+    if (comp) tc.n += n_plain;
+    const bool active = t.valid && (t.x0 + b * 8 < w);
+    const bool recompute = comp && !t_src;
+
+    f32x4 pre[6] = {};
+    fetch_strip(comp ? (t_src ? t_src : y_src) : x_plain, pre, t, h, w, lane);
+    bool fast1, fast2;
+    stage_tables_pair(q1, q2, qT1, qT2, fast1, fast2);
+
+    float px[24];
+    float tx[3][8];
+    float tg[3][8];
+    float none[1][8];
+    commit_strip(lds, pre, lane);
+    uint2 mm = make_uint2(0u, 0u);
+    if (!recompute) {
+        fetch_strip(gC, pre, tc, h, w, lane);
+        if (active) mm = *mask_row(mask2, tc, h, w, b, r);
+    }
+    wave_sync();
+    read_row24(lds, b, r, px);
+    wave_sync();
+    if (recompute) {
+        uint32_t mlo, mhi;
+        codec_rows<Q_RINT>(lds, qT1, fast1, active, t, b, r, hb, wb, nullptr, nullptr, px, mlo, mhi);
+        fetch_strip(gC, pre, tc, h, w, lane);
+        if (active) mm = *mask_row(mask2, tc, h, w, b, r);
+    }
+    grad_rows_x(px, tx);
+    commit_strip(lds, pre, lane);
+    wave_sync();
+    read_row24(lds, b, r, px);
+    wave_sync();
+    DJ_GRAD_ROWS_G(px, mm, tg)
+    grad_columns<GMODE2, QMODE2, false>(lds, qT2, fast2, active, b, r, tx, tg, none);
+    if (comp) {
+        fetch_strip(y_src, pre, t, h, w, lane);
+        mm = make_uint2(0u, 0u);
+        if (active) mm = *mask_row(mask1, t, h, w, b, r);
+    }
+    transpose24(lds, b, r, tg);
+    DJ_GRAD_ROWS_OUT(tg, px, lds, b, r)
+    if (comp) {
+        float pg[24];
+        wave_sync();
+        read_row24(lds, b, r, pg);
+        wave_sync();
+        commit_strip(lds, pre, lane);
+        wave_sync();
+        read_row24(lds, b, r, px);
+        wave_sync();
+        grad_rows_x(px, tx);
+        DJ_GRAD_ROWS_G(pg, mm, tg)
+        grad_columns<G_SOFT, Q_RINT, false>(lds, qT1, fast1, active, b, r, tx, tg, none);
+        transpose24(lds, b, r, tg);
+        DJ_GRAD_ROWS_OUT(tg, px, lds, b, r)
+    }
+    wave_sync();
+    store_strip(comp ? g_comp : g_plain, lds, t, h, w, lane);
+}
+
 inline int persistent_grid(long tasks) { return (int)((tasks + WAVES_PER_BLOCK - 1) / WAVES_PER_BLOCK); }
-constexpr size_t kLds = ((size_t)WAVES_PER_BLOCK * WAVE_LDS_F + 384 + 4) * sizeof(float);
+constexpr size_t kLds = ((size_t)WAVES_PER_BLOCK * WAVE_LDS_F + TABLES_F) * sizeof(float);
+constexpr size_t kLdsChain = kLds + TABLES_F * sizeof(float);
 
 template <bool DQ, typename... A>
 void launch_bwd(int rounding, int grid, hipStream_t s, A... a) {
@@ -240,6 +396,24 @@
         case NIMG_ROUND_HARMONIC: hipLaunchKernelGGL((djpeg_bwd_kernel<NIMG_ROUND_HARMONIC, DQ>), g, b, kLds, s, a...); break;
         default: hipLaunchKernelGGL((djpeg_bwd_kernel<NIMG_ROUND_IDENTITY, DQ>), g, b, kLds, s, a...); break;
     }
+}
+
+template <typename... A>
+void launch_chain_bwd(int rounding2, int grid, hipStream_t s, A... a) {
+    const dim3 g(grid), b(256);
+    switch (rounding2) {
+        case NIMG_ROUND_ROUND: hipLaunchKernelGGL((djpeg_chain_bwd_kernel<NIMG_ROUND_ROUND>), g, b, kLdsChain, s, a...); break;
+        case NIMG_ROUND_SIN:
+        case NIMG_ROUND_SOFT: hipLaunchKernelGGL((djpeg_chain_bwd_kernel<NIMG_ROUND_SOFT>), g, b, kLdsChain, s, a...); break;
+        case NIMG_ROUND_HARMONIC: hipLaunchKernelGGL((djpeg_chain_bwd_kernel<NIMG_ROUND_HARMONIC>), g, b, kLdsChain, s, a...); break;
+        default: hipLaunchKernelGGL((djpeg_chain_bwd_kernel<NIMG_ROUND_IDENTITY>), g, b, kLdsChain, s, a...); break;
+    }
+}
+
+inline bool chain_args_bad(int n_plain, int n_comp, int h, int w, int rounding1, int rounding2) {
+    if (n_plain < 0 || n_comp < 0 || h <= 0 || w <= 0 || (h % 8) || (w % 8)) return true;
+    if (rounding1 < NIMG_ROUND_ROUND || rounding1 > NIMG_ROUND_IDENTITY) return true;
+    return rounding2 < NIMG_ROUND_ROUND || rounding2 > NIMG_ROUND_IDENTITY;
 }
 
 }
@@ -281,6 +455,49 @@
     return NIMG_OK;
 }
 
+int nimg_djpeg_chain_fwd(const float* x_plain, const float* y_src, float* t_out, float* C, const float* q1, const float* q2,
+                         uint8_t* mask1, uint8_t* mask2, int n_plain, int n_comp, int h, int w, int rounding1, int rounding2,
+                         int shared, void* stream) {
+    if (n_plain == 0 && n_comp == 0) return NIMG_OK;
+    if (chain_args_bad(n_plain, n_comp, h, w, rounding1, rounding2)) return NIMG_ERR_ARG;
+    if (!C || !q1 || !q2 || (n_plain && !x_plain) || (n_comp && !y_src)) return NIMG_ERR_ARG;
+    if (fwd_mode(rounding1) != Q_RINT) return NIMG_ERR_ARG;
+    if (shared && (rounding1 != rounding2 || y_src != x_plain || n_comp > n_plain)) return NIMG_ERR_ARG;
+    const int first_plain = shared ? n_comp : 0;
+    const long tasks = (long)(n_comp + n_plain - first_plain) * (h / 8) * ((w + STRIP_PX - 1) / STRIP_PX);
+    const dim3 grid(persistent_grid(tasks)), block(256);
+    hipStream_t s = (hipStream_t)stream;
+    const int sh = shared ? 1 : 0;
+#define NIMG_CHAIN_FWD(Q)                                                                                                       \
+    hipLaunchKernelGGL(djpeg_chain_fwd_kernel<Q>, grid, block, kLdsChain, s, x_plain, y_src, t_out, C, q1, q2, mask1, mask2,     \
+                       n_plain, n_comp, first_plain, sh, h, w)
+    switch (fwd_mode(rounding2)) {
+        case Q_RINT: NIMG_CHAIN_FWD(Q_RINT); break;
+        case Q_SIN: NIMG_CHAIN_FWD(Q_SIN); break;
+        case Q_HARMONIC: NIMG_CHAIN_FWD(Q_HARMONIC); break;
+        default: NIMG_CHAIN_FWD(Q_IDENTITY); break;
+    }
+#undef NIMG_CHAIN_FWD
+    NIMG_CHECK_LAUNCH();
+    return NIMG_OK;
+}
+
+int nimg_djpeg_chain_bwd(const float* x_plain, const float* y_src, const float* t_src, const float* gC, const uint8_t* mask1,
+                         const uint8_t* mask2, const float* q1, const float* q2, float* g_plain, float* g_comp, int n_plain,
+                         int n_comp, int h, int w, int rounding1, int rounding2, int shared, void* stream) {
+    if (n_plain == 0 && n_comp == 0) return NIMG_OK;
+    if (chain_args_bad(n_plain, n_comp, h, w, rounding1, rounding2)) return NIMG_ERR_ARG;
+    if (!gC || !mask2 || !q1 || !q2 || (n_plain && (!x_plain || !g_plain)) || (n_comp && (!y_src || !mask1 || !g_comp)))
+        return NIMG_ERR_ARG;
+    if (rounding1 != NIMG_ROUND_SOFT) return NIMG_ERR_ARG;
+    if (shared && (rounding1 != rounding2 || !t_src)) return NIMG_ERR_ARG;
+    const long tasks = (long)(n_comp + n_plain) * (h / 8) * ((w + STRIP_PX - 1) / STRIP_PX);
+    launch_chain_bwd(rounding2, persistent_grid(tasks), (hipStream_t)stream, x_plain, y_src, t_src, gC, mask1, mask2, q1, q2,
+                     g_plain, g_comp, n_plain, n_comp, h, w);
+    NIMG_CHECK_LAUNCH();
+    return NIMG_OK;
+}
+
 size_t nimg_djpeg_dq_workspace_bytes(int n, int h, int w) {
     if (n <= 0 || h <= 0 || w <= 0) return 0;
     const long tasks = (long)n * (h / 8) * ((w + STRIP_PX - 1) / STRIP_PX);
diff --git a/neural-imaging_amd/models/jpeg.py b/neural-imaging_amd/models/jpeg.py
--- a/neural-imaging_amd/models/jpeg.py
+++ b/neural-imaging_amd/models/jpeg.py
@@ -23,6 +23,35 @@
     if _common_codec is None:
         _common_codec = JPEG(None, 'soft')
     return _common_codec.process(x, quality)
+
+
+CHAIN_COMPOSITE = True
+
+
+def chain_qualifies(manipulation, channel):
+    return CHAIN_COMPOSITE and all(isinstance(j, JPEG) and j._codec_model is not None and j._factors == (1, 1) and not j.trainable
+                                   for j in (manipulation, channel)) and manipulation.codec == 'soft'
+
+
+def chain_forward(manipulation, channel, x_plain, y_src, quality, training=False, t_out=None):
+    resolved1 = manipulation.resolve_quality(manipulation.quality if quality is None else quality)
+    resolved2 = channel.resolve_quality(channel.quality)
+    q1 = manipulation._codec_model.qtables(resolved1, x_plain.device)
+    q2 = channel._codec_model.qtables(resolved2, x_plain.device)
+    shared = resolved1 == resolved2 and manipulation.codec == channel.codec and y_src.data_ptr() == x_plain.data_ptr()
+    C, mask1, mask2 = ops.djpeg_chain_fwd(x_plain, y_src, q1, q2, manipulation.codec, channel.codec, shared=shared,
+                                          want_mask=training, t_out=t_out)
+    if not training:
+        return C, None
+    n = y_src.shape[0]
+    return C, {'x_plain': x_plain, 'y_src': y_src, 'q1': q1, 'q2': q2, 'mask1': mask2[:n] if shared else mask1, 'mask2': mask2,
+               'rounding': (manipulation.codec, channel.codec), 'shared': shared,
+               't_src': C[:n] if shared else t_out}
+
+
+def chain_backward(ctx, dC):
+    return ops.djpeg_chain_bwd(ctx['x_plain'], ctx['y_src'], dC, ctx['mask1'], ctx['mask2'], ctx['q1'], ctx['q2'],
+                               ctx['rounding'][0], ctx['rounding'][1], shared=ctx['shared'], t_src=ctx['t_src'])
 
 
 class DifferentiableJPEG(object):
diff --git a/neural-imaging_amd/ops.py b/neural-imaging_amd/ops.py
--- a/neural-imaging_amd/ops.py
+++ b/neural-imaging_amd/ops.py
@@ -458,6 +458,34 @@
     _lib.call('nimg_djpeg_bwd_dq', _p(x), _p(gy), _p(mask), _p(qtab), _p(gx), _p(dq), n, h, w, ROUNDING[rounding],
               1 if accumulate else 0, _p(ws), need, _stream())
     return gx
+
+
+def djpeg_chain_fwd(x_plain, y_src, q1, q2, rounding1='soft', rounding2='soft', shared=False, want_mask=True, t_out=None,
+                    out=None):
+    _f32(x_plain, y_src, q1, q2, t_out, out)
+    n_plain, h, w, c = x_plain.shape
+    n_comp = y_src.shape[0]
+    if c != 3 or tuple(y_src.shape[1:]) != (h, w, 3):
+        raise ValueError('dJPEG expects NHW3 images of one size')
+    C = torch.empty((n_plain + n_comp, h, w, 3), dtype=torch.float32, device=x_plain.device) if out is None else out
+    mask2 = torch.empty((n_plain + n_comp, h, w), dtype=torch.uint8, device=x_plain.device) if want_mask else None
+    mask1 = torch.empty((n_comp, h, w), dtype=torch.uint8, device=x_plain.device) if want_mask and not shared else None
+    _lib.call('nimg_djpeg_chain_fwd', _p(x_plain), _p(y_src), _p(t_out), _p(C), _p(q1), _p(q2), _p(mask1), _p(mask2),
+              n_plain, n_comp, h, w, ROUNDING[rounding1], ROUNDING[rounding2], 1 if shared else 0, _stream())
+    return C, mask1, mask2
+
+
+def djpeg_chain_bwd(x_plain, y_src, gC, mask1, mask2, q1, q2, rounding1='soft', rounding2='soft', shared=False, t_src=None):
+    _f32(x_plain, y_src, gC, q1, q2, t_src)
+    _chk(mask1, mask2)
+    n_plain, h, w, _ = x_plain.shape
+    n_comp = y_src.shape[0]
+    g_plain = torch.empty_like(x_plain)
+    g_comp = torch.empty_like(y_src)
+    _lib.call('nimg_djpeg_chain_bwd', _p(x_plain), _p(y_src), _p(t_src), _p(gC), _p(mask1), _p(mask2), _p(q1), _p(q2),
+              _p(g_plain), _p(g_comp), n_plain, n_comp, h, w, ROUNDING[rounding1], ROUNDING[rounding2], 1 if shared else 0,
+              _stream())
+    return g_plain, g_comp
 
 
 def _djpeg_sub_shape(x, hs, vs):
diff --git a/neural-imaging_amd/workflows/manipulation_classification.py b/neural-imaging_amd/workflows/manipulation_classification.py
--- a/neural-imaging_amd/workflows/manipulation_classification.py
+++ b/neural-imaging_amd/workflows/manipulation_classification.py
@@ -130,7 +130,12 @@
             self._labels_cache[batch_size] = torch.from_numpy(self._batch_labels(batch_size)).to(self.device)
         return self._labels_cache[batch_size]
 
-    def _manipulations(self, Y, randomize=False, override=None, training=False, m=None):
+    def _chains_jpeg(self, train_dcn=False):
+        names = list(self._operations.keys())
+        return bool(names) and names[-1] == 'jpeg' and self._distribution['downsampling'] == 'none' and \
+            self._distribution['compression'] == 'jpeg' and not train_dcn and jpeg.chain_qualifies(self._jpeg_manip, self.codec)
+
+    def _manipulations(self, Y, randomize=False, override=None, training=False, m=None, defer_jpeg=False):
         override = override if override is not None else self._strengths
         b = Y.shape[0]
         if m is None:
@@ -147,6 +152,9 @@
             strengths = override
         for k, (name, op) in enumerate(self._operations.items()):
             s = strengths[name]
+            if defer_jpeg and name == 'jpeg':
+                ctxs.append(s)
+                continue
             _, ctx = op.forward(Y, s, out=m[(k + 1) * b:(k + 2) * b], training=training)
             ctxs.append(ctx)
         return m, ctxs
@@ -186,9 +194,14 @@
         self.finish_pending()
         x = to_device(batch_x, self.device)
         Y = self.nip.forward(x)[0]
-        m, _ = self._manipulations(Y, augment)
-        c = self._downsampling(m)
-        C, ent, _ = self._codec_forward(c)
+        chained = self._chains_jpeg()
+        m, mctxs = self._manipulations(Y, augment, defer_jpeg=chained)
+        if chained:
+            c = m
+            C, ent = self._chain_forward(m, Y.shape[0], mctxs[-1], keep_manipulated=True)[0], None
+        else:
+            c = self._downsampling(m)
+            C, ent, _ = self._codec_forward(c)
         entropy = np.nan if ent is None else DeviceArray(ent)
         probs = self.fan.forward(C)[0]
         return DeviceArray(Y), DeviceArray(c), DeviceArray(C), entropy, DeviceArray(probs)
@@ -229,6 +242,11 @@
         C = torch.from_numpy(self.run_rgb_to_fan(batch_Y)).to(self.device)
         return self.fan.forward(C)[0].cpu().numpy()
 
+    def _chain_forward(self, m, b, strength, training=False, keep_manipulated=False):
+        k = self.n_classes - 1
+        return jpeg.chain_forward(self._jpeg_manip, self.codec, m[:k * b], m[:b], strength, training=training,
+                                  t_out=m[k * b:] if keep_manipulated else None)
+
     def _codec_forward(self, c, training=False):
         if self.codec is None:
             return c, None, None
@@ -255,9 +273,14 @@
             Y, nctx = self.nip.forward(x, training=train_nip, out=m[:b])
         else:
             Y, nctx = self.nip.forward(x, training=train_nip)
-        m, mctxs = self._manipulations(Y, augment, training=train_nip, m=m)
-        c = self._downsampling(m)
-        C, entropy, cctx = self._codec_forward(c, training=need_upstream)
+        chained = self._chains_jpeg(train_dcn)
+        m, mctxs = self._manipulations(Y, augment, training=train_nip, m=m, defer_jpeg=chained)
+        if chained:
+            c, entropy = m, None
+            C, cctx = self._chain_forward(m, b, mctxs[-1], training=need_upstream)
+        else:
+            c = self._downsampling(m)
+            C, entropy, cctx = self._codec_forward(c, training=need_upstream)
         self._finish_pending_fan()
         _, fctx = self.fan.forward(C, self._device_labels(b), training=True)
 
@@ -278,6 +301,8 @@
         if need_upstream:
             if self.codec is None:
                 dc = dC
+            elif chained:
+                dc, dY_jpeg = jpeg.chain_backward(cctx, dC)
             elif self._is_dcn:
                 lam = float(lambda_dcn) * world if train_dcn else 0.0
                 dc_direct = None
@@ -311,7 +336,7 @@
                     self._bucket.launch(self.codec._model.flat_grad)
         if train_nip:
             dm = self._downsampling_bwd(dc)
-            parts_dY = [dm[:b]] + [op.backward(mctxs[k], dm[(k + 1) * b:(k + 2) * b])
+            parts_dY = [dm[:b]] + [dY_jpeg if chained and name == 'jpeg' else op.backward(mctxs[k], dm[(k + 1) * b:(k + 2) * b])
                                    for k, (name, op) in enumerate(self._operations.items())]
             dY = dm[:b]
             head = self.nip.head_gradient(parts_dY, Y, target, float(lambda_nip)) if hasattr(self.nip, 'head_gradient') else None
```

Result: slower. 8287 patches/s (-2.1%).
